# michiyasunaga/qagnn

Measured on NVIDIA B200. Metric: GNN edges/sec, higher is better.
Workload: dtype f32

## Files before the change

### include/qagnn_b200.h

```cpp
#ifndef QAGNN_B200_H_
#define QAGNN_B200_H_

#include <stddef.h>
#include <stdint.h>

#ifdef __cplusplus
extern "C" {
#endif

#define QAGNN_ABI_VERSION 3

enum {
  QAGNN_OK = 0,
  QAGNN_ERR_INVALID_ARGUMENT = -1,
  QAGNN_ERR_CUDA = -2,
  QAGNN_ERR_INDEX_RANGE = -3,
  QAGNN_ERR_WORKSPACE = -4,
  QAGNN_ERR_UNSUPPORTED = -5
};

typedef struct qagnn_shape {
  int64_t N;
  int64_t E;
  int32_t D;
  int32_t H;
  int32_t T;
  int32_t R;
  int32_t k;
  int32_t n_per_graph;
} qagnn_shape;

typedef struct qagnn_edge_encoder_params {
  const float *lin0_w, *lin0_b;
  const float *bn_w, *bn_b, *bn_mean, *bn_var;
  const float *lin3_w, *lin3_b;
} qagnn_edge_encoder_params;

typedef struct qagnn_layer_params {
  const float *key_w, *key_b;
  const float *msg_w, *msg_b;
  const float *query_w, *query_b;
  const float *mlp0_w, *mlp0_b;
  const float *bn_w, *bn_b, *bn_mean, *bn_var;
  const float *mlp3_w, *mlp3_b;
} qagnn_layer_params;

typedef struct qagnn_mp_params {
  const float *emb_node_type_w, *emb_node_type_b;
  const float *emb_score_w, *emb_score_b;
  const float *vh_w, *vh_b, *vx_w, *vx_b;
  const float *score_basis;
} qagnn_mp_params;

int32_t qagnn_abi_version(void);
const char *qagnn_status_string(int32_t status);
const char *qagnn_last_cuda_error(void);


typedef struct qagnn_prep_layout {
  size_t total_bytes;
  size_t src;
  size_t tgt;
  size_t combo;
  size_t rowptr_src;
  size_t rowptr_tgt;
  size_t perm_src;
  size_t perm_tgt;
  size_t csr_src_tgt;
  size_t csr_src_combo;
  size_t csr_tgt_src;
  size_t csr_tgt_combo;
  size_t csr_tgt_apos;
  size_t pk_src;
  size_t pk_tgt;
  size_t csr_src_tpos;
  size_t order_src;
  size_t order_tgt;
  size_t ninfo_src;
  size_t ninfo_tgt;
  size_t status;
  size_t scratch;
} qagnn_prep_layout;

int32_t qagnn_graph_prep_layout(int64_t N, int64_t E, qagnn_prep_layout *out_host);
size_t qagnn_graph_prep_bytes(int64_t N, int64_t E);

int32_t qagnn_graph_prep(const int64_t *edge_index, const int64_t *edge_type, const int64_t *node_type,
                         const qagnn_shape *shape, void *prep, size_t prep_bytes, int32_t validate,
                         void *stream);

int32_t qagnn_graph_prep_packed(const int64_t *edge_index, const int64_t *edge_type, const int64_t *node_type,
                                const int64_t *graph_ptr, int32_t max_edges_per_graph, const qagnn_shape *shape, void *prep,
                                size_t prep_bytes, int32_t validate, void *stream);


size_t qagnn_fold_bytes(const qagnn_shape *shape);
int32_t qagnn_fold_weights(const qagnn_shape *shape, const qagnn_edge_encoder_params *edge_encoder_host,
                           const qagnn_layer_params *layers_host, const qagnn_mp_params *mp_host,
                           void *folded, size_t folded_bytes, void *stream);


size_t qagnn_forward_workspace_bytes(const qagnn_shape *shape);

int32_t qagnn_gatconve_forward(const qagnn_shape *shape, int32_t layer, const float *x, const float *extra,
                               const void *prep, const void *folded, float *out, float *alpha_out,
                               float *aggr_out, void *workspace, size_t workspace_bytes, void *stream);

int32_t qagnn_node_feature_extra(const qagnn_shape *shape, const int64_t *node_type, const float *node_score,
                                 const void *folded, float *extra_out, void *workspace, size_t workspace_bytes,
                                 void *stream);

int32_t qagnn_mp_forward(const qagnn_shape *shape, const float *H_in, const int64_t *node_type,
                         const float *node_score, const void *prep, const void *folded, float *out,
                         float *x_layers_out, void *workspace, size_t workspace_bytes, void *stream);


int32_t qagnn_mp_core_forward(const qagnn_shape *shape, const void *prep, const float *qkm, const float *ke, const float *me,
                              float *aggr, float *alpha_scaled, float *alpha_out, float *scratch, void *stream);

int32_t qagnn_mp_core_backward(const qagnn_shape *shape, const void *prep, const int32_t *combo_order, const float *qkm,
                               const float *ke, const float *me, const float *alpha_scaled, const float *d_aggr,
                               float *d_qkm, float *d_ke, float *d_me, float *scratch, void *stream);

size_t qagnn_linear_workspace_bytes(int64_t M, int32_t N, int32_t K1, int32_t K2);
int32_t qagnn_linear_bf16x3(const float *A1, int32_t lda1, int32_t K1, const float *A2, int32_t lda2, int32_t K2,
                            const float *W, int32_t ldw, const float *bias, float *C, int32_t ldc, int64_t M, int32_t N,
                            int32_t act, void *workspace, size_t workspace_bytes, void *stream);

int32_t qagnn_attention_pool(int32_t B, int32_t n, int32_t D, int32_t n_head, const float *X, const float *qs,
                             const uint8_t *mask, const float *wk, const float *bk, const float *wv, const float *bv,
                             float *pooled, float *attn, void *stream);

int32_t qagnn_decoder_tail(int32_t B, int32_t n, int32_t D, int32_t n_head, int32_t S, const float *X, const float *qs,
                           const int64_t *node_type, const int64_t *adj_lengths, const float *sent_vecs, const float *wk,
                           const float *bk, const float *wv, const float *bv, float *concat, float *attn, void *stream);

int32_t qagnn_decoder_head(int32_t B, int32_t n, int32_t D, const int64_t *concept_ids, int64_t n_concept, const float *table,
                           const float *ctx, const float *node_scores, const int64_t *adj_lengths, float *H_out,
                           float *scores_out, void *stream);

int64_t qagnn_launch_count(void);

enum {
  QAGNN_PROF_GRAPH_PREP = 0,
  QAGNN_PROF_PROJECTION = 1,
  QAGNN_PROF_MESSAGE_PASSING = 2,
  QAGNN_PROF_NODE_MLP = 3,
  QAGNN_PROF_PRO_EPILOGUE = 4,
  QAGNN_PROF_STAGES = 5
};
int32_t qagnn_profile_enable(int32_t on);
int32_t qagnn_profile_read(double *ms_out , int64_t *count_out );

#ifdef __cplusplus
}
#endif
#endif
```

### qagnn_b200/_lib.py

```python
import ctypes as C
import os

import torch

_HERE = os.path.dirname(os.path.abspath(__file__))
LIB_PATH = os.path.join(_HERE, "lib", "libqagnn_b200.so")

OK = 0
STATUS = {0: "ok", -1: "invalid argument", -2: "CUDA error", -3: "index out of range",
          -4: "workspace too small", -5: "unsupported shape"}


class Shape(C.Structure):
    _fields_ = [("N", C.c_int64), ("E", C.c_int64), ("D", C.c_int32), ("H", C.c_int32), ("T", C.c_int32),
                ("R", C.c_int32), ("k", C.c_int32), ("n_per_graph", C.c_int32)]


_P = C.c_void_p


class EdgeEncoderParams(C.Structure):
    _fields_ = [(n, _P) for n in ("lin0_w", "lin0_b", "bn_w", "bn_b", "bn_mean", "bn_var", "lin3_w", "lin3_b")]


class LayerParams(C.Structure):
    _fields_ = [(n, _P) for n in ("key_w", "key_b", "msg_w", "msg_b", "query_w", "query_b", "mlp0_w", "mlp0_b",
                                  "bn_w", "bn_b", "bn_mean", "bn_var", "mlp3_w", "mlp3_b")]


class MPParams(C.Structure):
    _fields_ = [(n, _P) for n in ("emb_node_type_w", "emb_node_type_b", "emb_score_w", "emb_score_b", "vh_w", "vh_b",
                                  "vx_w", "vx_b", "score_basis")]


class PrepLayout(C.Structure):
    _fields_ = [(n, C.c_size_t) for n in ("total_bytes", "src", "tgt", "combo", "rowptr_src", "rowptr_tgt", "perm_src",
                                          "perm_tgt", "csr_src_tgt", "csr_src_combo", "csr_tgt_src", "csr_tgt_combo",
                                          "csr_tgt_apos", "pk_src", "pk_tgt", "csr_src_tpos", "order_src", "order_tgt", "ninfo_src", "ninfo_tgt",
                                          "status", "scratch")]


EXPORTS = {
    "qagnn_abi_version": (C.c_int32, []),
    "qagnn_status_string": (C.c_char_p, [C.c_int32]),
    "qagnn_last_cuda_error": (C.c_char_p, []),
    "qagnn_graph_prep_layout": (C.c_int32, [C.c_int64, C.c_int64, C.POINTER(PrepLayout)]),
    "qagnn_graph_prep_bytes": (C.c_size_t, [C.c_int64, C.c_int64]),
    "qagnn_graph_prep": (C.c_int32, [_P, _P, _P, C.POINTER(Shape), _P, C.c_size_t, C.c_int32, _P]),
    "qagnn_graph_prep_packed": (C.c_int32, [_P, _P, _P, _P, C.c_int32, C.POINTER(Shape), _P, C.c_size_t, C.c_int32, _P]),
    "qagnn_fold_bytes": (C.c_size_t, [C.POINTER(Shape)]),
    "qagnn_fold_weights": (C.c_int32, [C.POINTER(Shape), C.POINTER(EdgeEncoderParams), C.POINTER(LayerParams),
                                       C.POINTER(MPParams), _P, C.c_size_t, _P]),
    "qagnn_forward_workspace_bytes": (C.c_size_t, [C.POINTER(Shape)]),
    "qagnn_gatconve_forward": (C.c_int32, [C.POINTER(Shape), C.c_int32, _P, _P, _P, _P, _P, _P, _P, _P, C.c_size_t, _P]),
    "qagnn_node_feature_extra": (C.c_int32, [C.POINTER(Shape), _P, _P, _P, _P, _P, C.c_size_t, _P]),
    "qagnn_mp_forward": (C.c_int32, [C.POINTER(Shape), _P, _P, _P, _P, _P, _P, _P, _P, C.c_size_t, _P]),
    "qagnn_mp_core_forward": (C.c_int32, [C.POINTER(Shape), _P, _P, _P, _P, _P, _P, _P, _P, _P]),
    "qagnn_mp_core_backward": (C.c_int32, [C.POINTER(Shape), _P, _P, _P, _P, _P, _P, _P, _P, _P, _P, _P, _P]),
    "qagnn_linear_workspace_bytes": (C.c_size_t, [C.c_int64, C.c_int32, C.c_int32, C.c_int32]),
    "qagnn_linear_bf16x3": (C.c_int32, [_P, C.c_int32, C.c_int32, _P, C.c_int32, C.c_int32, _P, C.c_int32, _P, _P, C.c_int32,
                                        C.c_int64, C.c_int32, C.c_int32, _P, C.c_size_t, _P]),
    "qagnn_attention_pool": (C.c_int32, [C.c_int32, C.c_int32, C.c_int32, C.c_int32, _P, _P, _P, _P, _P, _P, _P, _P, _P, _P]),
    "qagnn_decoder_tail": (C.c_int32, [C.c_int32, C.c_int32, C.c_int32, C.c_int32, C.c_int32, _P, _P, _P, _P, _P, _P, _P, _P, _P, _P,
                                       _P, _P]),
    "qagnn_decoder_head": (C.c_int32, [C.c_int32, C.c_int32, C.c_int32, _P, C.c_int64, _P, _P, _P, _P, _P, _P, _P]),
    "qagnn_launch_count": (C.c_int64, []),
    "qagnn_profile_enable": (C.c_int32, [C.c_int32]),
    "qagnn_profile_read": (C.c_int32, [C.POINTER(C.c_double), C.POINTER(C.c_int64)]),
}

_lib = None


def load():
    global _lib
    if _lib is not None:
        return _lib
    from . import build as _build
    if not _build.is_current():
        import fcntl
        stale = os.path.exists(LIB_PATH)
        try:
            _build._nvcc()
        except RuntimeError:
            raise RuntimeError(
                f"{LIB_PATH} is {'older than qagnn_b200/csrc' if stale else 'missing'} and there is no nvcc to build it. Run "
                f"`python -c 'import __graft_entry__ as g; g.build()'` on a machine with the CUDA toolkit. There is no CPU fallback.") from None
        os.makedirs(os.path.dirname(LIB_PATH), exist_ok=True)
        with open(LIB_PATH + ".lock", "w") as lock:
            fcntl.flock(lock, fcntl.LOCK_EX)
            try:
                if not _build.is_current():
                    _build.build()
            except Exception as e:
                raise RuntimeError(f"{LIB_PATH} is {'older than qagnn_b200/csrc' if stale else 'missing'} and could not be "
                                   f"built: {e}. There is no CPU fallback.") from e
            finally:
                fcntl.flock(lock, fcntl.LOCK_UN)
    if not os.path.exists(LIB_PATH):
        raise RuntimeError(f"{LIB_PATH} is missing after a build. There is no CPU fallback.")
    lib = C.CDLL(LIB_PATH)
    for name, (res, args) in EXPORTS.items():
        fn = getattr(lib, name)
        fn.restype, fn.argtypes = res, args
    if lib.qagnn_abi_version() != 3:
        raise RuntimeError("libqagnn_b200.so ABI version mismatch")
    _lib = lib
    return lib


PROF_STAGES = ("graph_prep", "projection", "message_passing", "node_mlp", "pro_epilogue")


def profile_read():
    lib = load()
    ms = (C.c_double * len(PROF_STAGES))()
    cnt = (C.c_int64 * len(PROF_STAGES))()
    check(lib.qagnn_profile_read(ms, cnt), "qagnn_profile_read")
    return {n: (ms[i], cnt[i]) for i, n in enumerate(PROF_STAGES)}


class QagnnError(RuntimeError):
    pass


def check(status, what):
    if status != OK:
        lib = load()
        msg = lib.qagnn_status_string(status).decode()
        if status == -2:
            msg += ": " + lib.qagnn_last_cuda_error().decode()
        if status == -3:
            raise IndexError(f"{what}: {msg}")
        raise QagnnError(f"{what}: {msg} (status {status})")


def ptr(t):
    return None if t is None else C.c_void_p(t.data_ptr())


def stream_ptr(device):
    return C.c_void_p(torch.cuda.current_stream(device).cuda_stream)


def require_cuda(t, name):
    if not t.is_cuda:
        raise RuntimeError(f"qagnn_b200: `{name}` must live on a CUDA device (got {t.device}); "
                           f"this implementation has no CPU path")


def f32c(t, name):
    require_cuda(t, name)
    if t.dtype != torch.float32:
        raise TypeError(f"qagnn_b200: `{name}` must be float32 (got {t.dtype})")
    return t.detach().contiguous()


def i64c(t, name):
    require_cuda(t, name)
    if t.dtype != torch.int64:
        raise TypeError(f"qagnn_b200: `{name}` must be int64 (got {t.dtype})")
    return t.contiguous()
```

### qagnn_b200/csrc/abi.cu

```cuda
#include <atomic>
#include <mutex>
#include <cuda_bf16.h>
#include <stdio.h>
#include <stdlib.h>
#include <string.h>

#include "common.cuh"

namespace qagnn {

static std::atomic<long long> g_launches{0};
static thread_local char g_cuda_err[256] = "";

void note_launch(int n) { g_launches.fetch_add(n, std::memory_order_relaxed); }

int32_t cuda_fail(cudaError_t e, const char* file, int line) {
  const char* base = strrchr(file, '/');
  snprintf(g_cuda_err, sizeof(g_cuda_err), "%s (%s:%d)", cudaGetErrorString(e), base ? base + 1 : file, line);
  return QAGNN_ERR_CUDA;
}

namespace {
constexpr int kProfMax = 8192;
struct ProfState {
  bool on = false;
  int n = 0;
  cudaEvent_t ev[kProfMax][2];
  int created = 0;
  int stage[kProfMax];
  int open_idx[QAGNN_PROF_STAGES];
  std::mutex mu;
} g_prof;
}

void prof_begin(int stage, cudaStream_t st) {
  if (!g_prof.on) return;
  std::lock_guard<std::mutex> lk(g_prof.mu);
  if (!g_prof.on || g_prof.n >= kProfMax) { if (g_prof.on) g_prof.open_idx[stage] = -1; return; }
  const int i = g_prof.n++;
  if (i >= g_prof.created) {
    cudaEventCreate(&g_prof.ev[i][0]);
    cudaEventCreate(&g_prof.ev[i][1]);
    g_prof.created = i + 1;
  }
  g_prof.stage[i] = stage;
  g_prof.open_idx[stage] = i;
  cudaEventRecord(g_prof.ev[i][0], st);
}

void prof_end(int stage, cudaStream_t st) {
  if (!g_prof.on) return;
  std::lock_guard<std::mutex> lk(g_prof.mu);
  const int i = g_prof.open_idx[stage];
  if (i >= 0) cudaEventRecord(g_prof.ev[i][1], st);
}

WorkLayout make_work_layout(const qagnn_shape& s) {
  WorkLayout W;
  const size_t N = (size_t)s.N, D = (size_t)s.D, Ep = (size_t)(s.N + s.E), H = (size_t)s.H;
  size_t o = 0;
  auto take = [&](size_t n) { size_t r = o; o += align_up(n * 4) / 4; return r; };
  const size_t DP = (size_t)head_dim_padded((int)(D / H));
  W.qkm = take(N * 3 * (D > H * DP ? D : H * DP));
  W.aggr = take(N * D);
  W.hmid = take(N * D);
  W.xa = take(N * D);
  W.xb = take(N * D);
  W.extra = take(N * D);
  W.sinb = take(N * (D / 2));
  const size_t half = N * D / 2 + 8;
  W.hp_hi = take(half); W.hp_lo = take(half);
  W.ep_hi = take(half); W.ep_lo = take(half);
  W.xp_hi[0] = take(half); W.xp_lo[0] = take(half);
  W.xp_hi[1] = take(half); W.xp_lo[1] = take(half);
  W.ap_hi = take(half); W.ap_lo = take(half);
  W.mp_hi = take(half); W.mp_lo = take(half);
  const size_t sbh = N * (size_t)round_up8((int)(D / 2)) / 2 + 8;
  W.sb_hi = take(sbh); W.sb_lo = take(sbh);
  const size_t xsh = N * (size_t)round_up8((int)(D + D / 2)) / 2 + 8;
  for (int i = 0; i < 3; ++i) { W.xs_hi[i] = take(xsh); W.xs_lo[i] = take(xsh); }
  const size_t Eps = (Ep + 3) / 4 * 4;
  W.score = take(Eps * H);
  W.alpha = take(Eps * H);
  W.alpha2 = take(2 * Eps * H);
  W.total = o;
  return W;
}

namespace {

__global__ void node_feature_prologue_kernel(int64_t N, int D, int T, const int64_t* __restrict__ node_type,
                                             const float* __restrict__ node_score, const float* __restrict__ type_tab,
                                             const float* __restrict__ basis, float* __restrict__ extra,
                                             float* __restrict__ sinb) {
  const int Dh = D / 2;
  for (int64_t i = blockIdx.x * (int64_t)blockDim.x + threadIdx.x; i < N * Dh; i += (int64_t)gridDim.x * blockDim.x) {
    const int64_t v = i / Dh;
    const int j = (int)(i % Dh);
    int64_t t = node_type[v];
    t = t < 0 ? 0 : (t >= T ? T - 1 : t);
    extra[v * D + j] = type_tab[t * Dh + j];
    sinb[i] = sinf(basis[j] * node_score[v]);
  }
}

__global__ void sin_basis_planes_kernel(int64_t N, int Dh, int ld, const float* __restrict__ node_score,
                                        const float* __restrict__ basis, __nv_bfloat16* __restrict__ hi,
                                        __nv_bfloat16* __restrict__ lo) {
  const int half = Dh / 2;
  for (int64_t i = blockIdx.x * (int64_t)blockDim.x + threadIdx.x; i < N * half; i += (int64_t)gridDim.x * blockDim.x) {
    const int64_t v = i / half;
    const int j = (int)(i % half) * 2;
    const float sc = node_score[v];
    const float a = sinf(basis[j] * sc), b = sinf(basis[j + 1] * sc);
    __nv_bfloat162 h2, l2;
    h2.x = __float2bfloat16_rn(a); h2.y = __float2bfloat16_rn(b);
    l2.x = __float2bfloat16_rn(a - __bfloat162float(h2.x)); l2.y = __float2bfloat16_rn(b - __bfloat162float(h2.y));
    *reinterpret_cast<__nv_bfloat162*>(hi + v * ld + j) = h2;
    *reinterpret_cast<__nv_bfloat162*>(lo + v * ld + j) = l2;
  }
}

__global__ void copy_plane_columns_kernel(int64_t N, int w4, int ld8, const uint2* __restrict__ sh, const uint2* __restrict__ sl,
                                          uint2* __restrict__ d1h, uint2* __restrict__ d1l, uint2* __restrict__ d2h,
                                          uint2* __restrict__ d2l) {
  for (int64_t i = blockIdx.x * (int64_t)blockDim.x + threadIdx.x; i < N * w4; i += (int64_t)gridDim.x * blockDim.x) {
    const int64_t r = i / w4;
    const int c = (int)(i - r * w4);
    const uint2 h = sh[r * ld8 + c], l = sl[r * ld8 + c];
    d1h[r * ld8 + c] = h; d1l[r * ld8 + c] = l;
    d2h[r * ld8 + c] = h; d2l[r * ld8 + c] = l;
  }
}

constexpr int kNfNodes = 64;
__global__ void __launch_bounds__(256) node_feature_fused_kernel(int64_t N, int D, int T, const int64_t* __restrict__ node_type,
                                                                  const float* __restrict__ node_score,
                                                                  const float* __restrict__ type_tab, const float* __restrict__ basis,
                                                                  const float* __restrict__ ws, const float* __restrict__ bs,
                                                                  float* __restrict__ extra, __nv_bfloat16* __restrict__ ex_hi,
                                                                  __nv_bfloat16* __restrict__ ex_lo) {
  extern __shared__ __align__(16) float sm_nf[];
  const int Dh = D / 2;
  float* Wt = sm_nf;
  float* Bt = Wt + (size_t)Dh * Dh;
  const int64_t v0 = (int64_t)blockIdx.x * kNfNodes;
  for (int i = threadIdx.x; i < Dh * Dh; i += 256) Wt[(i % Dh) * Dh + i / Dh] = ws[i];
  for (int i = threadIdx.x; i < kNfNodes * Dh; i += 256) {
    const int k = i / kNfNodes, vi = i % kNfNodes;
    const int64_t v = v0 + vi;
    Bt[i] = v < N ? sinf(basis[k] * node_score[v]) : 0.f;
  }
  __syncthreads();
  auto put4 = [&](int64_t v, int col, const float (&x)[4]) {
    if (extra != nullptr) *reinterpret_cast<float4*>(extra + v * D + col) = make_float4(x[0], x[1], x[2], x[3]);
    if (ex_hi != nullptr) {
      __nv_bfloat16 h[4], l[4];
#pragma unroll
      for (int c = 0; c < 4; ++c) {
        h[c] = __float2bfloat16_rn(x[c]);
        l[c] = __float2bfloat16_rn(x[c] - __bfloat162float(h[c]));
      }
      *reinterpret_cast<uint2*>(ex_hi + v * D + col) = *reinterpret_cast<const uint2*>(h);
      *reinterpret_cast<uint2*>(ex_lo + v * D + col) = *reinterpret_cast<const uint2*>(l);
    }
  };
  const int jg = Dh / 4, ntile = (kNfNodes / 4) * jg;
  for (int tl = threadIdx.x; tl < ntile; tl += 256) {
    const int vi0 = (tl / jg) * 4, j0 = (tl % jg) * 4;
    float acc[4][4];
#pragma unroll
    for (int a = 0; a < 4; ++a)
#pragma unroll
      for (int c = 0; c < 4; ++c) acc[a][c] = 0.f;
    for (int k = 0; k < Dh; ++k) {
      const float4 b = *reinterpret_cast<const float4*>(Bt + k * kNfNodes + vi0);
      const float4 w = *reinterpret_cast<const float4*>(Wt + k * Dh + j0);
      const float bb[4] = {b.x, b.y, b.z, b.w}, ww[4] = {w.x, w.y, w.z, w.w};
#pragma unroll
      for (int a = 0; a < 4; ++a)
#pragma unroll
        for (int c = 0; c < 4; ++c) acc[a][c] = fmaf(bb[a], ww[c], acc[a][c]);
    }
#pragma unroll
    for (int a = 0; a < 4; ++a) {
      const int64_t v = v0 + vi0 + a;
      if (v >= N) continue;
      int64_t t = node_type[v];
      t = t < 0 ? 0 : (t >= T ? T - 1 : t);
      float sc[4], ty[4];
#pragma unroll
      for (int c = 0; c < 4; ++c) {
        sc[c] = gelu_tanh(acc[a][c] + bs[j0 + c]);
        ty[c] = type_tab[t * Dh + j0 + c];
      }
      put4(v, Dh + j0, sc);
      put4(v, j0, ty);
    }
  }
}

int32_t check_shape_fwd(const qagnn_shape* s) {
  if (!s) return QAGNN_ERR_INVALID_ARGUMENT;
  if (s->N <= 0 || s->E < 0 || s->D <= 0 || s->H <= 0 || s->T <= 0 || s->R <= 0 || s->k < 0)
    return QAGNN_ERR_INVALID_ARGUMENT;
  if (s->D % s->H != 0 || s->D % 2 != 0) return QAGNN_ERR_INVALID_ARGUMENT;
  if (s->N + s->E >= (int64_t)1 << 31) return QAGNN_ERR_INVALID_ARGUMENT;
  return QAGNN_OK;
}

bool use_headtile(const qagnn_shape& s) {
  const char* e = getenv("QAGNN_MP_PATH");
  const bool forced = e && (strcmp(e, "csr") == 0 || strcmp(e, "basic") == 0);
  return !forced && headtile_supported(s);
}
bool use_slice(const qagnn_shape& s) {
  const char* e = getenv("QAGNN_MP_PATH");
  return !(e && strcmp(e, "basic") == 0) && slice_supported(s);
}
bool mp_path_supported(const qagnn_shape& s) { return use_headtile(s) || use_slice(s) || basic_mp_supported(s); }

int32_t layer_forward(const qagnn_shape& s, const FoldLayout& L, const WorkLayout& W, int layer, const float* x,
                      const float* extra, const void* prep, const qagnn_prep_layout& pl, const float* folded,
                      float* out, float* alpha_out, float* aggr_out, float* ws, Act final_act, bool tiled,
                      cudaStream_t st) {
  const int D = s.D;
  const float* lb = folded + L.layer0 + (size_t)layer * L.layer_stride;
  float* qkm = ws + W.qkm;
  float* aggr = aggr_out ? aggr_out : ws + W.aggr;
  {
    ProfScope ps(QAGNN_PROF_PROJECTION, st);
    HeadMajorOut hm{tiled ? 1 : 0, D, D / s.H, head_dim_padded(D / s.H), s.H};
    QAGNN_RETURN_IF(sgemm_tn(x, D, D, extra, D, D, lb + L.wp, 2 * D, lb + L.bp, qkm, 3 * D, s.N, 3 * D, ACT_NONE, st, hm));
  }
  {
    ProfScope ps(QAGNN_PROF_MESSAGE_PASSING, st);
    if (tiled) {
      QAGNN_RETURN_IF(launch_message_passing_headtile(s, (const int32_t*)prep, pl, qkm, lb + L.keh, lb + L.meh,
                                                      ws + W.score, ws + W.alpha2, aggr, alpha_out, nullptr, nullptr, st));
    } else if (use_slice(s)) {
      QAGNN_RETURN_IF(launch_message_passing_slice(s, (const int32_t*)prep, pl, qkm, lb + L.ke, lb + L.me, ws + W.score, aggr,
                                                   alpha_out, st));
    } else {
      QAGNN_RETURN_IF(launch_message_passing(s, (const int32_t*)prep, pl, qkm, lb + L.ke, lb + L.me, ws + W.score,
                                             ws + W.alpha, aggr, alpha_out, st));
    }
  }
  {
    ProfScope ps(QAGNN_PROF_NODE_MLP, st);
    QAGNN_RETURN_IF(sgemm_tn(aggr, D, D, nullptr, 0, 0, lb + L.w1, D, lb + L.b1, ws + W.hmid, D, s.N, D, ACT_RELU, st));
    QAGNN_RETURN_IF(sgemm_tn(ws + W.hmid, D, D, nullptr, 0, 0, lb + L.w2, D, lb + L.b2, out, D, s.N, D, final_act, st));
  }
  return QAGNN_OK;
}

bool use_tc(const qagnn_shape& s) { return gemm_tc_available() && s.D % 8 == 0; }

struct Planes {
  const void* hi;
  const void* lo;
  int ld = 0;
};

int32_t layer_forward_tc(const qagnn_shape& s, const FoldLayout& L, const WorkLayout& W, int layer, Planes x, Planes extra,
                         const void* prep, const qagnn_prep_layout& pl, const float* folded, float* out_f32,
                         void* out_hi, void* out_lo, float* alpha_out, float* aggr_out, float* ws, Act final_act,
                         bool tiled, cudaStream_t st, const int64_t* type_bias_classes = nullptr, int out_ldp = 0) {
  const int D = s.D;
  if (out_ldp == 0) out_ldp = D;
  const float* lb = folded + L.layer0 + (size_t)layer * L.layer_stride;
  float* qkm = ws + W.qkm;
  const bool fused_split = tiled && (D / s.H) % 2 == 0;
  float* aggr = aggr_out ? aggr_out : (fused_split ? nullptr : ws + W.aggr);
  {
    ProfScope ps(QAGNN_PROF_PROJECTION, st);
    TcOperand A1{x.hi, x.lo, x.ld ? x.ld : D, D}, A2{extra.hi, extra.lo, D, D};
    TcOutput o{};
    if (tiled && type_bias_classes != nullptr) {
      const int DP = head_dim_padded(D / s.H), KS = round_up8(D + D / 2);
      TcOperand Ax{x.hi, x.lo, KS, D + D / 2}, none{nullptr, nullptr, 0, 0};
      TcOperand Wp{lb + L.wps_hi, lb + L.wps_lo, KS, D + D / 2};
      o.hm_buf = qkm;
      o.hm = HeadMajorOut{1, D, D / s.H, DP, s.H};
      o.row_class = type_bias_classes; o.class_stride = 3 * s.H * DP; o.n_class = s.T;
      QAGNN_RETURN_IF(gemm_tc(Ax, none, Wp, lb + L.tbias, s.N, 3 * s.H * DP, ACT_NONE, o, st));
    } else if (tiled) {
      const int DP = head_dim_padded(D / s.H);
      TcOperand Wp{lb + L.wph_hi, lb + L.wph_lo, 2 * D, 2 * D};
      o.hm_buf = qkm;
      o.hm = HeadMajorOut{1, D, D / s.H, DP, s.H};
      QAGNN_RETURN_IF(gemm_tc(A1, A2, Wp, lb + L.bph, s.N, 3 * s.H * DP, ACT_NONE, o, st));
    } else {
      TcOperand Wp{lb + L.wp_hi, lb + L.wp_lo, 2 * D, 2 * D};
      o.f32 = qkm;
      o.ldc = 3 * D;
      QAGNN_RETURN_IF(gemm_tc(A1, A2, Wp, lb + L.bp, s.N, 3 * D, ACT_NONE, o, st));
    }
  }
  {
    ProfScope ps(QAGNN_PROF_MESSAGE_PASSING, st);
    if (tiled) {
      QAGNN_RETURN_IF(launch_message_passing_headtile(s, (const int32_t*)prep, pl, qkm, lb + L.keh, lb + L.meh,
                                                      ws + W.score, ws + W.alpha2, aggr, alpha_out,
                                                      fused_split ? ws + W.ap_hi : nullptr, ws + W.ap_lo, st));
    } else if (use_slice(s)) {
      QAGNN_RETURN_IF(launch_message_passing_slice(s, (const int32_t*)prep, pl, qkm, lb + L.ke, lb + L.me, ws + W.score, aggr,
                                                   alpha_out, st));
    } else {
      QAGNN_RETURN_IF(launch_message_passing(s, (const int32_t*)prep, pl, qkm, lb + L.ke, lb + L.me, ws + W.score,
                                             ws + W.alpha, aggr, alpha_out, st));
    }
  }
  {
    ProfScope ps(QAGNN_PROF_NODE_MLP, st);
    if (!fused_split) QAGNN_RETURN_IF(split_bf16(aggr, D, s.N, D, ws + W.ap_hi, ws + W.ap_lo, D, st));
    TcOperand A{ws + W.ap_hi, ws + W.ap_lo, D, D}, none{nullptr, nullptr, 0, 0};
    TcOperand W1{lb + L.w1_hi, lb + L.w1_lo, D, D}, W2{lb + L.w2_hi, lb + L.w2_lo, D, D};
    TcOutput o1{};
    o1.hi = ws + W.mp_hi; o1.lo = ws + W.mp_lo; o1.ldp = D;
    QAGNN_RETURN_IF(gemm_tc(A, none, W1, lb + L.b1, s.N, D, ACT_RELU, o1, st));
    TcOperand Hm{ws + W.mp_hi, ws + W.mp_lo, D, D};
    TcOutput o2{};
    o2.f32 = out_f32; o2.ldc = D; o2.hi = out_hi; o2.lo = out_lo; o2.ldp = out_ldp;
    QAGNN_RETURN_IF(gemm_tc(Hm, none, W2, lb + L.b2, s.N, D, final_act, o2, st));
  }
  return QAGNN_OK;
}

int32_t extra_forward(const qagnn_shape& s, const FoldLayout& L, const WorkLayout& W, const int64_t* node_type,
                      const float* node_score, const float* folded, float* extra, float* ws, cudaStream_t st,
                      void* ex_hi = nullptr, void* ex_lo = nullptr) {
  ProfScope ps(QAGNN_PROF_PRO_EPILOGUE, st);
  const int D = s.D, Dh = D / 2;
  if (Dh <= 128 && D % 8 == 0) {
    const size_t smem = ((size_t)Dh * Dh + (size_t)kNfNodes * Dh) * sizeof(float);
    static size_t attr[kMaxDevices] = {0};
    const int dev = current_device();
    if (smem > 48 * 1024 && smem > attr[dev]) {
      QAGNN_CHECK_CUDA(cudaFuncSetAttribute(node_feature_fused_kernel, cudaFuncAttributeMaxDynamicSharedMemorySize, (int)smem));
      attr[dev] = smem;
    }
    node_feature_fused_kernel<<<(unsigned)((s.N + kNfNodes - 1) / kNfNodes), 256, smem, st>>>(
        s.N, D, s.T, node_type, node_score, folded + L.type_tab, folded + L.basis, folded + L.ws, folded + L.bs, extra,
        (__nv_bfloat16*)ex_hi, (__nv_bfloat16*)ex_lo);
    QAGNN_CHECK_LAUNCH();
    return QAGNN_OK;
  }
  const int64_t n = s.N * Dh;
  int64_t g = (n + 255) / 256;
  if (g > 148 * 32) g = 148 * 32;
  node_feature_prologue_kernel<<<(unsigned)g, 256, 0, st>>>(s.N, D, s.T, node_type, node_score, folded + L.type_tab,
                                                            folded + L.basis, extra, ws + W.sinb);
  QAGNN_CHECK_LAUNCH();
  QAGNN_RETURN_IF(sgemm_tn(ws + W.sinb, Dh, Dh, nullptr, 0, 0, folded + L.ws, Dh, folded + L.bs, extra + Dh, D, s.N, Dh,
                           ACT_GELU, st));
  if (ex_hi != nullptr) QAGNN_RETURN_IF(split_bf16(extra, D, s.N, D, ex_hi, ex_lo, D, st));
  return QAGNN_OK;
}

}
}

using namespace qagnn;

extern "C" int32_t qagnn_abi_version(void) { return QAGNN_ABI_VERSION; }

extern "C" const char* qagnn_status_string(int32_t status) {
  switch (status) {
    case QAGNN_OK: return "ok";
    case QAGNN_ERR_INVALID_ARGUMENT: return "invalid argument";
    case QAGNN_ERR_CUDA: return "CUDA error";
    case QAGNN_ERR_INDEX_RANGE: return "index out of range in edge_index / edge_type / node_type";
    case QAGNN_ERR_WORKSPACE: return "workspace too small";
    case QAGNN_ERR_UNSUPPORTED: return "unsupported shape";
    default: return "unknown status";
  }
}

extern "C" const char* qagnn_last_cuda_error(void) { return g_cuda_err; }

extern "C" int64_t qagnn_launch_count(void) { return (int64_t)g_launches.load(std::memory_order_relaxed); }

extern "C" int32_t qagnn_profile_enable(int32_t on) {
  std::lock_guard<std::mutex> lk(g_prof.mu);
  g_prof.on = on != 0;
  g_prof.n = 0;
  for (int i = 0; i < QAGNN_PROF_STAGES; ++i) g_prof.open_idx[i] = -1;
  return QAGNN_OK;
}

extern "C" int32_t qagnn_profile_read(double* ms_out, int64_t* count_out) {
  if (!ms_out || !count_out) return QAGNN_ERR_INVALID_ARGUMENT;
  std::lock_guard<std::mutex> lk(g_prof.mu);
  for (int i = 0; i < QAGNN_PROF_STAGES; ++i) { ms_out[i] = 0.0; count_out[i] = 0; }
  for (int i = 0; i < g_prof.n; ++i) {
    QAGNN_CHECK_CUDA(cudaEventSynchronize(g_prof.ev[i][1]));
    float ms = 0.f;
    QAGNN_CHECK_CUDA(cudaEventElapsedTime(&ms, g_prof.ev[i][0], g_prof.ev[i][1]));
    ms_out[g_prof.stage[i]] += ms;
    count_out[g_prof.stage[i]] += 1;
  }
  return QAGNN_OK;
}

extern "C" size_t qagnn_forward_workspace_bytes(const qagnn_shape* shape) {
  if (check_shape_fwd(shape) != QAGNN_OK) return 0;
  return align_up(make_work_layout(*shape).total * sizeof(float));
}

extern "C" int32_t qagnn_gatconve_forward(const qagnn_shape* shape, int32_t layer, const float* x, const float* extra,
                                          const void* prep, const void* folded, float* out, float* alpha_out,
                                          float* aggr_out, void* workspace, size_t workspace_bytes, void* stream) {
  QAGNN_RETURN_IF(check_shape_fwd(shape));
  if (!x || !extra || !prep || !folded || !out || !workspace) return QAGNN_ERR_INVALID_ARGUMENT;
  if (layer < 0 || layer >= shape->k) return QAGNN_ERR_INVALID_ARGUMENT;
  if (!mp_path_supported(*shape)) return QAGNN_ERR_UNSUPPORTED;
  const FoldLayout L = make_fold_layout(*shape);
  const WorkLayout W = make_work_layout(*shape);
  if (workspace_bytes < W.total * sizeof(float)) return QAGNN_ERR_WORKSPACE;
  qagnn_prep_layout pl;
  QAGNN_RETURN_IF(qagnn_graph_prep_layout(shape->N, shape->E, &pl));
  const bool tiled = use_headtile(*shape);
  cudaStream_t st = (cudaStream_t)stream;
  float* ws = (float*)workspace;
  if (tiled && !use_tc(*shape)) QAGNN_RETURN_IF(zero_head_pads(*shape, ws + W.qkm, st));
  if (use_tc(*shape)) {
    const int D = shape->D;
    QAGNN_RETURN_IF(split_bf16(x, D, shape->N, D, ws + W.xp_hi[0], ws + W.xp_lo[0], D, st));
    QAGNN_RETURN_IF(split_bf16(extra, D, shape->N, D, ws + W.ep_hi, ws + W.ep_lo, D, st));
    return layer_forward_tc(*shape, L, W, layer, Planes{ws + W.xp_hi[0], ws + W.xp_lo[0]}, Planes{ws + W.ep_hi, ws + W.ep_lo},
                            prep, pl, (const float*)folded, out, nullptr, nullptr, alpha_out, aggr_out, ws, ACT_NONE, tiled, st);
  }
  return layer_forward(*shape, L, W, layer, x, extra, prep, pl, (const float*)folded, out, alpha_out, aggr_out, ws,
                       ACT_NONE, tiled, st);
}

extern "C" int32_t qagnn_node_feature_extra(const qagnn_shape* shape, const int64_t* node_type, const float* node_score,
                                            const void* folded, float* extra_out, void* workspace,
                                            size_t workspace_bytes, void* stream) {
  QAGNN_RETURN_IF(check_shape_fwd(shape));
  if (!node_type || !node_score || !folded || !extra_out || !workspace) return QAGNN_ERR_INVALID_ARGUMENT;
  const FoldLayout L = make_fold_layout(*shape);
  const WorkLayout W = make_work_layout(*shape);
  if (workspace_bytes < W.total * sizeof(float)) return QAGNN_ERR_WORKSPACE;
  return extra_forward(*shape, L, W, node_type, node_score, (const float*)folded, extra_out, (float*)workspace,
                       (cudaStream_t)stream);
}

extern "C" int32_t qagnn_mp_forward(const qagnn_shape* shape, const float* H_in, const int64_t* node_type,
                                    const float* node_score, const void* prep, const void* folded, float* out,
                                    float* x_layers_out, void* workspace, size_t workspace_bytes, void* stream) {
  QAGNN_RETURN_IF(check_shape_fwd(shape));
  if (!H_in || !node_type || !node_score || !prep || !folded || !out || !workspace) return QAGNN_ERR_INVALID_ARGUMENT;
  const qagnn_shape& s = *shape;
  if (s.k > 0 && !mp_path_supported(s)) return QAGNN_ERR_UNSUPPORTED;
  const FoldLayout L = make_fold_layout(s);
  const WorkLayout W = make_work_layout(s);
  if (workspace_bytes < W.total * sizeof(float)) return QAGNN_ERR_WORKSPACE;
  qagnn_prep_layout pl;
  QAGNN_RETURN_IF(qagnn_graph_prep_layout(s.N, s.E, &pl));
  cudaStream_t st = (cudaStream_t)stream;
  float* ws = (float*)workspace;
  const float* f = (const float*)folded;
  float* extra = ws + W.extra;
  const bool tc = use_tc(s);
  const bool tiled = use_headtile(s);
  const char* efp = getenv("QAGNN_MP_FASTPROJ");
  const bool fast = tc && tiled && s.k > 0 && (s.D / 2) % 4 == 0 && !(efp && atoi(efp) == 0);
  if (fast) {
    const int D = s.D, Dh = D / 2, KSh = round_up8(Dh), KS = round_up8(D + Dh);
    char* xh[3]; char* xl[3];
    for (int i = 0; i < 3; ++i) { xh[i] = (char*)(ws + W.xs_hi[i]); xl[i] = (char*)(ws + W.xs_lo[i]); }
    {
      ProfScope ps(QAGNN_PROF_PRO_EPILOGUE, st);
      int64_t g = (s.N * (Dh / 2) + 255) / 256;
      if (g > 148 * 32) g = 148 * 32;
      sin_basis_planes_kernel<<<(unsigned)g, 256, 0, st>>>(s.N, Dh, KSh, node_score, f + L.basis, (__nv_bfloat16*)(ws + W.sb_hi),
                                                           (__nv_bfloat16*)(ws + W.sb_lo));
      QAGNN_CHECK_LAUNCH();
      TcOperand A{ws + W.sb_hi, ws + W.sb_lo, KSh, Dh}, none{nullptr, nullptr, 0, 0}, Wsc{f + L.ws_hi, f + L.ws_lo, KSh, Dh};
      TcOutput o{};
      o.hi = xh[0] + (size_t)D * 2; o.lo = xl[0] + (size_t)D * 2; o.ldp = KS;
      QAGNN_RETURN_IF(gemm_tc(A, none, Wsc, f + L.bs, s.N, Dh, ACT_GELU, o, st));
      {
        const int w4 = Dh * 2 / 8, ld8 = KS * 2 / 8;
        int64_t gc = (s.N * w4 + 255) / 256;
        if (gc > 148 * 16) gc = 148 * 16;
        const size_t off = (size_t)D * 2;
        copy_plane_columns_kernel<<<(unsigned)gc, 256, 0, st>>>(s.N, w4, ld8, (const uint2*)(xh[0] + off), (const uint2*)(xl[0] + off),
                                                              (uint2*)(xh[1] + off), (uint2*)(xl[1] + off), (uint2*)(xh[2] + off),
                                                              (uint2*)(xl[2] + off));
        QAGNN_CHECK_LAUNCH();
      }
      QAGNN_RETURN_IF(split_bf16(H_in, D, s.N, D, xh[0], xl[0], KS, st));
    }
    const size_t ND = (size_t)s.N * s.D;
    Planes xin{xh[0], xl[0], KS};
    const Planes ep{nullptr, nullptr, 0};
    for (int l = 0; l < s.k; ++l) {
      float* xo32 = x_layers_out ? x_layers_out + (size_t)l * ND : nullptr;
      void* ohi = xh[1 + (l & 1)];
      void* olo = xl[1 + (l & 1)];
      QAGNN_RETURN_IF(layer_forward_tc(s, L, W, l, xin, ep, prep, pl, f, xo32, ohi, olo, nullptr, nullptr, ws, ACT_GELU, tiled, st,
                                       node_type, KS));
      xin = Planes{ohi, olo, KS};
    }
    ProfScope ps(QAGNN_PROF_PRO_EPILOGUE, st);
    TcOperand A1{xh[0], xl[0], KS, D}, A2{xin.hi, xin.lo, KS, D}, Wv{f + L.vcat_hi, f + L.vcat_lo, 2 * D, 2 * D};
    TcOutput o{};
    o.f32 = out; o.ldc = D;
    return gemm_tc(A1, A2, Wv, f + L.vbias, s.N, D, ACT_GELU, o, st);
  }
  {
    QAGNN_RETURN_IF(extra_forward(s, L, W, node_type, node_score, f, tc && s.D / 2 <= 128 ? nullptr : extra, ws, st,
                                  tc ? ws + W.ep_hi : nullptr, tc ? ws + W.ep_lo : nullptr));
  }
  if (tiled && !use_tc(s)) QAGNN_RETURN_IF(zero_head_pads(s, ws + W.qkm, st));
  const size_t ND = (size_t)s.N * s.D;
  if (tc) {
    const int D = s.D;
    {
      ProfScope ps(QAGNN_PROF_PRO_EPILOGUE, st);
      QAGNN_RETURN_IF(split_bf16(H_in, D, s.N, D, ws + W.hp_hi, ws + W.hp_lo, D, st));
    }
    Planes xin{ws + W.hp_hi, ws + W.hp_lo};
    const Planes ep{ws + W.ep_hi, ws + W.ep_lo};
    for (int l = 0; l < s.k; ++l) {
      float* xo32 = x_layers_out ? x_layers_out + (size_t)l * ND : nullptr;
      void* ohi = ws + W.xp_hi[l & 1];
      void* olo = ws + W.xp_lo[l & 1];
      QAGNN_RETURN_IF(layer_forward_tc(s, L, W, l, xin, ep, prep, pl, f, xo32, ohi, olo, nullptr, nullptr, ws, ACT_GELU,
                                       tiled, st));
      xin = Planes{ohi, olo};
    }
    ProfScope ps(QAGNN_PROF_PRO_EPILOGUE, st);
    TcOperand A1{ws + W.hp_hi, ws + W.hp_lo, D, D}, A2{xin.hi, xin.lo, D, D}, Wv{f + L.vcat_hi, f + L.vcat_lo, 2 * D, 2 * D};
    TcOutput o{};
    o.f32 = out; o.ldc = D;
    if (s.k == 0) { A2 = A1; }
    return gemm_tc(A1, A2, Wv, f + L.vbias, s.N, D, ACT_GELU, o, st);
  }
  const float* x = H_in;
  for (int l = 0; l < s.k; ++l) {
    float* xo = x_layers_out ? x_layers_out + (size_t)l * ND : ws + ((l & 1) ? W.xb : W.xa);
    QAGNN_RETURN_IF(layer_forward(s, L, W, l, x, extra, prep, pl, f, xo, nullptr, nullptr, ws, ACT_GELU, tiled, st));
    x = xo;
  }
  ProfScope ps(QAGNN_PROF_PRO_EPILOGUE, st);
  return sgemm_tn(H_in, s.D, s.D, x, s.D, s.D, f + L.vcat, 2 * s.D, f + L.vbias, out, s.D, s.N, s.D, ACT_GELU, st);
}

extern "C" int32_t qagnn_mp_core_forward(const qagnn_shape* shape, const void* prep, const float* qkm, const float* ke,
                                         const float* me, float* aggr, float* alpha_scaled, float* alpha_out, float* scratch,
                                         void* stream) {
  QAGNN_RETURN_IF(check_shape_fwd(shape));
  if (!prep || !qkm || !ke || !me || !aggr || !alpha_scaled || !scratch) return QAGNN_ERR_INVALID_ARGUMENT;
  qagnn_prep_layout pl;
  QAGNN_RETURN_IF(qagnn_graph_prep_layout(shape->N, shape->E, &pl));
  cudaStream_t st = (cudaStream_t)stream;
  ProfScope ps(QAGNN_PROF_MESSAGE_PASSING, st);
  return launch_message_passing(*shape, (const int32_t*)prep, pl, qkm, ke, me, scratch, alpha_scaled, aggr, alpha_out, st);
}

extern "C" int32_t qagnn_mp_core_backward(const qagnn_shape* shape, const void* prep, const int32_t* combo_order,
                                          const float* qkm, const float* ke, const float* me, const float* alpha_scaled,
                                          const float* d_aggr, float* d_qkm, float* d_ke, float* d_me, float* scratch,
                                          void* stream) {
  QAGNN_RETURN_IF(check_shape_fwd(shape));
  if (!prep || !combo_order || !qkm || !ke || !me || !alpha_scaled || !d_aggr || !d_qkm || !d_ke || !d_me || !scratch)
    return QAGNN_ERR_INVALID_ARGUMENT;
  qagnn_prep_layout pl;
  QAGNN_RETURN_IF(qagnn_graph_prep_layout(shape->N, shape->E, &pl));
  return launch_message_passing_backward(*shape, (const int32_t*)prep, pl, combo_order, qkm, ke, me, alpha_scaled, d_aggr,
                                         scratch, d_qkm, d_ke, d_me, (cudaStream_t)stream);
}

extern "C" size_t qagnn_linear_workspace_bytes(int64_t M, int32_t N, int32_t K1, int32_t K2) {
  if (M <= 0 || N <= 0 || K1 <= 0 || K2 < 0) return 0;
  const size_t K = (size_t)K1 + K2;
  return align_up(2 * 2 * ((size_t)M * K + (size_t)N * K) + 8 * 1024);
}

extern "C" int32_t qagnn_linear_bf16x3(const float* A1, int32_t lda1, int32_t K1, const float* A2, int32_t lda2, int32_t K2,
                                       const float* Wt, int32_t ldw, const float* bias, float* C, int32_t ldc, int64_t M,
                                       int32_t N, int32_t act, void* workspace, size_t workspace_bytes, void* stream) {
  if (!A1 || !Wt || !C || !workspace || M <= 0 || N <= 0 || K1 <= 0 || K2 < 0 || (K2 > 0 && !A2)) return QAGNN_ERR_INVALID_ARGUMENT;
  if (act < 0 || act > 2) return QAGNN_ERR_INVALID_ARGUMENT;
  if (workspace_bytes < qagnn_linear_workspace_bytes(M, N, K1, K2)) return QAGNN_ERR_WORKSPACE;
  if (!gemm_tc_available() || !gemm_tc_shape_ok(K1, K2, K1, K2, K1 + K2, N)) return QAGNN_ERR_UNSUPPORTED;
  cudaStream_t st = (cudaStream_t)stream;
  char* w = (char*)workspace;
  auto take = [&](size_t elems) { char* r = w; w += align_up(elems * 2); return (void*)r; };
  const int K = K1 + K2;
  void *a1h = take((size_t)M * K1), *a1l = take((size_t)M * K1);
  void *a2h = K2 ? take((size_t)M * K2) : nullptr, *a2l = K2 ? take((size_t)M * K2) : nullptr;
  void *wh = take((size_t)N * K), *wl = take((size_t)N * K);
  QAGNN_RETURN_IF(split_bf16(A1, lda1, M, K1, a1h, a1l, K1, st));
  if (K2) QAGNN_RETURN_IF(split_bf16(A2, lda2, M, K2, a2h, a2l, K2, st));
  QAGNN_RETURN_IF(split_bf16(Wt, ldw, N, K, wh, wl, K, st));
  TcOperand o1{a1h, a1l, K1, K1}, o2{a2h, a2l, K2, K2}, ow{wh, wl, K, K};
  TcOutput out{};
  out.f32 = C;
  out.ldc = ldc;
  return gemm_tc(o1, o2, ow, bias, M, N, (Act)act, out, st);
}
```

### qagnn_b200/csrc/common.cuh

```cuda
#pragma once

#include <cuda_runtime.h>
#include <stddef.h>
#include <stdint.h>

#include "../../include/qagnn_b200.h"

namespace qagnn {

constexpr size_t kAlign = 256;
__host__ __device__ inline size_t align_up(size_t x, size_t a = kAlign) { return (x + a - 1) / a * a; }

void note_launch(int n = 1);
int32_t cuda_fail(cudaError_t e, const char* file, int line);

#define QAGNN_CHECK_LAUNCH()                               \
  do {                                                     \
    cudaError_t e__ = cudaGetLastError();                  \
    if (e__ != cudaSuccess) return ::qagnn::cuda_fail(e__, __FILE__, __LINE__);\
    ::qagnn::note_launch();                                \
  } while (0)

#define QAGNN_CHECK_CUDA(expr)                              \
  do {                                                     \
    cudaError_t e__ = (expr);                              \
    if (e__ != cudaSuccess) return ::qagnn::cuda_fail(e__, __FILE__, __LINE__);\
  } while (0)

#define QAGNN_RETURN_IF(st)        \
  do {                             \
    int32_t s__ = (st);            \
    if (s__ != QAGNN_OK) return s__; \
  } while (0)

constexpr int kMaxDevices = 64;
inline int current_device() {
  int dev = 0;
  if (cudaGetDevice(&dev) != cudaSuccess || dev < 0 || dev >= kMaxDevices) dev = 0;
  return dev;
}

void prof_begin(int stage, cudaStream_t st);
void prof_end(int stage, cudaStream_t st);
struct ProfScope {
  int stage; cudaStream_t st;
  ProfScope(int s, cudaStream_t t) : stage(s), st(t) { prof_begin(stage, st); }
  ~ProfScope() { prof_end(stage, st); }
};

struct FoldLayout {
  int D, H, T, R, k, C;
  size_t tab;
  size_t hidden;
  size_t type_tab;
  size_t basis;
  size_t ws;
  size_t bs;
  size_t vcat;
  size_t vbias;
  size_t layer0;
  size_t layer_stride;
  size_t wp;
  size_t bp;
  size_t ke;
  size_t me;
  size_t w1;
  size_t b1;
  size_t w2;
  size_t b2;
  size_t keh;
  size_t meh;
  size_t wp_hi, wp_lo;
  size_t wph, bph;
  size_t wph_hi, wph_lo;
  size_t w1_hi, w1_lo;
  size_t w2_hi, w2_lo;
  size_t vcat_hi, vcat_lo;
  size_t ws_hi, ws_lo;
  size_t wps;
  size_t wps_hi, wps_lo;
  size_t tbias;
  size_t total;
};
FoldLayout make_fold_layout(const qagnn_shape& s);

struct WorkLayout {
  size_t qkm;
  size_t aggr;
  size_t hmid;
  size_t xa, xb;
  size_t extra;
  size_t sinb;
  size_t hp_hi, hp_lo;
  size_t ep_hi, ep_lo;
  size_t xp_hi[2], xp_lo[2];
  size_t ap_hi, ap_lo;
  size_t mp_hi, mp_lo;
  size_t sb_hi, sb_lo;
  size_t xs_hi[3], xs_lo[3];
  size_t score;
  size_t alpha;
  size_t alpha2;
  size_t total;
};
WorkLayout make_work_layout(const qagnn_shape& s);

enum Act { ACT_NONE = 0, ACT_RELU = 1, ACT_GELU = 2 };

struct HeadMajorOut {
  int enabled, D, d, DP, H;
};

int32_t sgemm_tn(const float* A1, int lda1, int K1, const float* A2, int lda2, int K2, const float* W, int ldw,
                 const float* bias, float* C, int ldc, int64_t M, int N, Act act, cudaStream_t st,
                 HeadMajorOut hm = HeadMajorOut{0, 0, 0, 0, 0});

struct TcOperand {
  const void* hi;
  const void* lo;
  int ld, K;
};
struct TcOutput {
  float* f32; int ldc;
  float* hm_buf; HeadMajorOut hm;
  void* hi; void* lo; int ldp;
  const int64_t* row_class; int class_stride; int n_class;
};
bool gemm_tc_available();
bool gemm_tc_shape_ok(int K1, int K2, int lda1, int lda2, int ldw, int N);
int32_t split_bf16(const float* a, int lda, long long M, int K, void* hi, void* lo, int ldp, cudaStream_t st);
int32_t gemm_tc(const TcOperand& A1, const TcOperand& A2, const TcOperand& W, const float* bias, long long M, int N,
                Act act, const TcOutput& out, cudaStream_t st);

inline int head_dim_padded(int d) { return (d + 3) / 4 * 4; }
inline int round_up8(int k) { return (k + 7) / 8 * 8; }
bool headtile_supported(const qagnn_shape& s);
int32_t launch_message_passing_headtile(const qagnn_shape& s, const int32_t* prep_base, const qagnn_prep_layout& pl,
                                        const float* qkmh, const float* keh, const float* meh, float* score,
                                        float* alpha2, float* aggr, float* alpha_out, void* aggr_hi, void* aggr_lo,
                                        cudaStream_t st);
int32_t zero_head_pads(const qagnn_shape& s, float* qkmh, cudaStream_t st);

bool basic_mp_supported(const qagnn_shape& s);
int32_t launch_message_passing(const qagnn_shape& s, const int32_t* prep_base, const qagnn_prep_layout& pl,
                               const float* qkm, const float* ke, const float* me, float* score, float* alpha,
                               float* aggr, float* alpha_out, cudaStream_t st);

bool slice_supported(const qagnn_shape& s);
int32_t launch_message_passing_slice(const qagnn_shape& s, const int32_t* prep_base, const qagnn_prep_layout& pl,
                                     const float* qkm, const float* ke, const float* me, float* score, float* aggr,
                                     float* alpha_out, cudaStream_t st);

int32_t launch_message_passing_backward(const qagnn_shape& s, const int32_t* prep_base, const qagnn_prep_layout& pl,
                                        const int32_t* combo_order, const float* qkm, const float* ke, const float* me,
                                        const float* alpha_s, const float* d_aggr, float* ds, float* d_qkm, float* d_ke,
                                        float* d_me, cudaStream_t st);

__device__ __forceinline__ float gelu_tanh(float x) {
  const float k0 = 0.7978845608028654f;
  return 0.5f * x * (1.0f + tanhf(k0 * (x + 0.044715f * x * x * x)));
}

}
```

### qagnn_b200/csrc/gemm_tc.cu

```cuda
#include <cuda.h>
#include <cuda_bf16.h>
#include <stdio.h>
#include <stdlib.h>
#include <string.h>

#include "common.cuh"

namespace qagnn {

namespace {

constexpr int BM = 128;
constexpr int kEpiWarps = 8;
constexpr int kThreads = (kEpiWarps + 2) * 32;
constexpr int kTmaWarp = kEpiWarps, kMmaWarp = kEpiWarps + 1;

struct alignas(64) TcParams {
  CUtensorMap a_hi[2], a_lo[2], w_hi, w_lo;
  CUtensorMap o_f32, o_hm, o_hi, o_lo;
  int nseg, kseg[2];
  int umma_n, n_step, N, stages;
  int nkb_total;
  long long M;
  const float* bias;
  const int64_t* row_class;
  int class_stride, n_class;
  int act;
  float* c_f32;
  int ldc;
  float* c_hm;
  HeadMajorOut hm;
  __nv_bfloat16 *c_hi, *c_lo;
  int ldp;
  unsigned tmem_cols;
};

__device__ __forceinline__ uint32_t smem_u32(const void* p) { return (uint32_t)__cvta_generic_to_shared(p); }

__device__ __forceinline__ void mbar_init(uint64_t* bar, uint32_t count) {
  asm volatile("mbarrier.init.shared::cta.b64 [%0], %1;" ::"r"(smem_u32(bar)), "r"(count) : "memory");
}
__device__ __forceinline__ void mbar_expect_tx(uint64_t* bar, uint32_t bytes) {
  asm volatile("mbarrier.arrive.expect_tx.shared::cta.b64 _, [%0], %1;" ::"r"(smem_u32(bar)), "r"(bytes) : "memory");
}
__device__ __forceinline__ void mbar_wait(uint64_t* bar, uint32_t parity) {
  uint32_t done;
  do {
    asm volatile(
        "{\n\t.reg .pred p;\n\t"
        "mbarrier.try_wait.parity.shared::cta.b64 p, [%1], %2;\n\t"
        "selp.u32 %0, 1, 0, p;\n\t}"
        : "=r"(done)
        : "r"(smem_u32(bar)), "r"(parity)
        : "memory");
  } while (!done);
}
__device__ __forceinline__ void tma_load_2d(void* dst, const CUtensorMap* map, int c0, int c1, uint64_t* bar) {
  asm volatile(
      "cp.async.bulk.tensor.2d.shared::cluster.global.tile.mbarrier::complete_tx::bytes [%0], [%1, {%2, %3}], [%4];" ::"r"(
          smem_u32(dst)),
      "l"(map), "r"(c0), "r"(c1), "r"(smem_u32(bar))
      : "memory");
}
__device__ __forceinline__ void tc_fence_before() { asm volatile("tcgen05.fence::before_thread_sync;" ::: "memory"); }
__device__ __forceinline__ void tc_fence_after() { asm volatile("tcgen05.fence::after_thread_sync;" ::: "memory"); }

template <int BK>
__device__ __forceinline__ uint64_t umma_desc(uint32_t saddr) {
  const uint32_t lo = ((saddr & 0x3FFFFu) >> 4) | (1u << 16);
  const uint32_t hi = (uint32_t)(8 * BK * 2 / 16) | (1u << 14) | ((BK == 64 ? 2u : 4u) << 29);
  return ((uint64_t)hi << 32) | lo;
}
__device__ __forceinline__ void umma_bf16(uint32_t tmem_d, uint64_t da, uint64_t db, uint32_t idesc, uint32_t acc) {
  asm volatile(
      "{\n\t.reg .pred p;\n\t"
      "setp.ne.b32 p, %4, 0;\n\t"
      "tcgen05.mma.cta_group::1.kind::f16 [%0], %1, %2, %3, p;\n\t}" ::"r"(tmem_d),
      "l"(da), "l"(db), "r"(idesc), "r"(acc)
      : "memory");
}
__device__ __forceinline__ void umma_commit(uint64_t* bar) {
  asm volatile("tcgen05.commit.cta_group::1.mbarrier::arrive::one.shared::cluster.b64 [%0];" ::"r"(smem_u32(bar)) : "memory");
}
__device__ __forceinline__ void tmem_ld32(uint32_t taddr, float (&v)[32]) {
  uint32_t r[32];
  asm volatile(
      "tcgen05.ld.sync.aligned.32x32b.x32.b32 "
      "{%0,%1,%2,%3,%4,%5,%6,%7,%8,%9,%10,%11,%12,%13,%14,%15,%16,%17,%18,%19,%20,%21,%22,%23,%24,%25,%26,%27,%28,%29,%30,%31}, [%32];"
      : "=r"(r[0]), "=r"(r[1]), "=r"(r[2]), "=r"(r[3]), "=r"(r[4]), "=r"(r[5]), "=r"(r[6]), "=r"(r[7]), "=r"(r[8]),
        "=r"(r[9]), "=r"(r[10]), "=r"(r[11]), "=r"(r[12]), "=r"(r[13]), "=r"(r[14]), "=r"(r[15]), "=r"(r[16]), "=r"(r[17]),
        "=r"(r[18]), "=r"(r[19]), "=r"(r[20]), "=r"(r[21]), "=r"(r[22]), "=r"(r[23]), "=r"(r[24]), "=r"(r[25]), "=r"(r[26]),
        "=r"(r[27]), "=r"(r[28]), "=r"(r[29]), "=r"(r[30]), "=r"(r[31])
      : "r"(taddr));
  asm volatile("tcgen05.wait::ld.sync.aligned;" ::: "memory");
#pragma unroll
  for (int i = 0; i < 32; ++i) v[i] = __uint_as_float(r[i]);
}

__device__ __forceinline__ float gelu_tanh_fast(float x) {
  const float u = 0.7978845608028654f * (x + 0.044715f * x * x * x);
  const float t = 1.f - __fdividef(2.f, __expf(2.f * u) + 1.f);
  return 0.5f * x * (1.f + t);
}

constexpr int kStageBytesPerWarp = 4096;

__device__ __forceinline__ void tma_store_2d(const CUtensorMap* map, int c0, int c1, const void* src) {
  asm volatile("cp.async.bulk.tensor.2d.global.shared::cta.tile.bulk_group [%0, {%1, %2}], [%3];" ::"l"(map), "r"(c0), "r"(c1),
               "r"(smem_u32(src))
               : "memory");
}
__device__ __forceinline__ void tma_store_3d(const CUtensorMap* map, int c0, int c1, int c2, const void* src) {
  asm volatile("cp.async.bulk.tensor.3d.global.shared::cta.tile.bulk_group [%0, {%1, %2, %3}], [%4];" ::"l"(map), "r"(c0),
               "r"(c1), "r"(c2), "r"(smem_u32(src))
               : "memory");
}
__device__ __forceinline__ void tma_store_commit() { asm volatile("cp.async.bulk.commit_group;" ::: "memory"); }
__device__ __forceinline__ void tma_store_wait_read() { asm volatile("cp.async.bulk.wait_group.read 0;" ::: "memory"); }
__device__ __forceinline__ void tma_store_wait_all() { asm volatile("cp.async.bulk.wait_group 0;" ::: "memory"); }

constexpr uint32_t kPeerBitMask = 0xFEFFFFFFu;
__device__ __forceinline__ uint32_t cluster_ctarank() {
  uint32_t r;
  asm volatile("mov.u32 %0, %%cluster_ctarank;" : "=r"(r));
  return r;
}
__device__ __forceinline__ void cluster_sync_all() {
  asm volatile("barrier.cluster.arrive.release.aligned;" ::: "memory");
  asm volatile("barrier.cluster.wait.acquire.aligned;" ::: "memory");
}
__device__ __forceinline__ void tma_load_2d_2sm(void* dst, const CUtensorMap* map, int c0, int c1, uint64_t* bar) {
  asm volatile(
      "cp.async.bulk.tensor.2d.cta_group::2.shared::cluster.global.mbarrier::complete_tx::bytes [%0], [%1, {%2, %3}], [%4];" ::"r"(
          smem_u32(dst)),
      "l"(map), "r"(c0), "r"(c1), "r"(smem_u32(bar) & kPeerBitMask)
      : "memory");
}
__device__ __forceinline__ void umma_bf16_2sm(uint32_t tmem_d, uint64_t da, uint64_t db, uint32_t idesc, uint32_t acc) {
  asm volatile(
      "{\n\t.reg .pred p;\n\t"
      "setp.ne.b32 p, %4, 0;\n\t"
      "tcgen05.mma.cta_group::2.kind::f16 [%0], %1, %2, %3, p;\n\t}" ::"r"(tmem_d),
      "l"(da), "l"(db), "r"(idesc), "r"(acc)
      : "memory");
}
__device__ __forceinline__ void umma_commit_2sm(uint64_t* bar) {
  asm volatile("tcgen05.commit.cta_group::2.mbarrier::arrive::one.shared::cluster.multicast::cluster.b64 [%0], %1;" ::"r"(smem_u32(bar)),
               "h"((uint16_t)3)
               : "memory");
}
__device__ __forceinline__ void mbar_arrive_leader(uint64_t* bar) {
  asm volatile("mbarrier.arrive.shared::cluster.b64 _, [%0];" ::"r"(smem_u32(bar) & kPeerBitMask) : "memory");
}

template <int ACT, int BK, int CTAS, bool WRES>
__global__ void __launch_bounds__(kThreads, 1) gemm_tc_kernel(const __grid_constant__ TcParams p) {
  extern __shared__ __align__(1024) unsigned char smem[];
  const int warp = threadIdx.x >> 5, lane = threadIdx.x & 31;
  const uint32_t a_bytes = BM * BK * 2;
  const uint32_t wn = (uint32_t)p.umma_n / CTAS;
  const uint32_t w_bytes = wn * BK * 2;
  const uint32_t stage_bytes = WRES ? 2 * a_bytes : 2 * a_bytes + 2 * w_bytes;
  const uint32_t rank = CTAS == 2 ? cluster_ctarank() : 0u;
  const bool leader = rank == 0;
  const unsigned cl_id = blockIdx.x / CTAS, n_cl = gridDim.x / CTAS;
  const uint32_t wres_bytes = WRES ? (uint32_t)p.nkb_total * 2u * w_bytes : 0u;
  unsigned char* wres = smem + (size_t)p.stages * stage_bytes;
  unsigned char* ctrl = wres + wres_bytes;
  uint64_t* full = reinterpret_cast<uint64_t*>(ctrl);
  uint64_t* empty = full + p.stages;
  uint64_t* acc_full = empty + p.stages;
  uint64_t* acc_empty = acc_full + 2;
  uint64_t* wfull = acc_empty + 2;
  uint32_t* tmem_slot = reinterpret_cast<uint32_t*>(wfull + 1);

  int nkb_seg[2];
  nkb_seg[0] = (p.kseg[0] + BK - 1) / BK;
  nkb_seg[1] = p.nseg > 1 ? (p.kseg[1] + BK - 1) / BK : 0;
  const int nkb = nkb_seg[0] + nkb_seg[1];
  const int n_tiles = (p.N + p.n_step - 1) / p.n_step;
  const long long m_tiles = (p.M + BM * CTAS - 1) / (BM * CTAS);
  const long long total_tiles = m_tiles * n_tiles;
  const int my_n = WRES ? (int)(cl_id % (unsigned)n_tiles) : 0;
  const long long w_idx = cl_id / (unsigned)n_tiles;
  const long long w_cnt = WRES ? ((long long)n_cl - my_n + n_tiles - 1) / n_tiles : 1;
  const long long t_first = WRES ? w_idx * n_tiles + my_n : (long long)cl_id;
  const long long t_step = WRES ? w_cnt * n_tiles : (long long)n_cl;

  if (threadIdx.x == 0) {
    for (int s = 0; s < p.stages; ++s) {
      mbar_init(&full[s], 1);
      mbar_init(&empty[s], 1);
    }
    for (int a = 0; a < 2; ++a) {
      mbar_init(&acc_full[a], 1);
      mbar_init(&acc_empty[a], kEpiWarps * CTAS);
    }
    mbar_init(wfull, 1);
    asm volatile("fence.mbarrier_init.release.cluster;" ::: "memory");
  }
  if (warp == kMmaWarp) {
    if (CTAS == 1) {
      asm volatile("tcgen05.alloc.cta_group::1.sync.aligned.shared::cta.b32 [%0], %1;" ::"r"(smem_u32(tmem_slot)), "r"(512u) : "memory");
      asm volatile("tcgen05.relinquish_alloc_permit.cta_group::1.sync.aligned;" ::: "memory");
    } else {
      asm volatile("tcgen05.alloc.cta_group::2.sync.aligned.shared::cta.b32 [%0], %1;" ::"r"(smem_u32(tmem_slot)), "r"(512u) : "memory");
      asm volatile("tcgen05.relinquish_alloc_permit.cta_group::2.sync.aligned;" ::: "memory");
    }
  }
  tc_fence_before();
  __syncthreads();
  if (CTAS == 2) cluster_sync_all();
  tc_fence_after();
  const uint32_t tmem_base = *tmem_slot;

  if (warp == kTmaWarp) {
    if (lane == 0) {
      long long it = 0;
      if (WRES && t_first < total_tiles) {
        const int n0 = my_n * p.n_step + (int)(rank * wn);
        if (CTAS == 1) mbar_expect_tx(wfull, wres_bytes);
        else if (leader) mbar_expect_tx(wfull, 2 * wres_bytes);
        for (int kb = 0; kb < nkb; ++kb) {
          unsigned char* dst = wres + (size_t)kb * 2 * w_bytes;
          if (CTAS == 1) {
            tma_load_2d(dst, &p.w_hi, kb * BK, n0, wfull);
            tma_load_2d(dst + w_bytes, &p.w_lo, kb * BK, n0, wfull);
          } else {
            tma_load_2d_2sm(dst, &p.w_hi, kb * BK, n0, wfull);
            tma_load_2d_2sm(dst + w_bytes, &p.w_lo, kb * BK, n0, wfull);
          }
        }
      }
      for (long long tile = t_first; tile < total_tiles; tile += t_step) {
        const int n0 = (int)(tile % n_tiles) * p.n_step + (int)(rank * wn);
        const int m0 = (int)((tile / n_tiles) * BM * CTAS + rank * BM);
        for (int kb = 0; kb < nkb; ++kb, ++it) {
          const int s = (int)(it % p.stages);
          if (it >= p.stages) mbar_wait(&empty[s], (uint32_t)((it / p.stages) - 1) & 1u);
          const int seg = kb < nkb_seg[0] ? 0 : 1;
          const int k_in_seg = (seg == 0 ? kb : kb - nkb_seg[0]) * BK;
          const int k_glob = (seg == 0 ? 0 : p.kseg[0]) + k_in_seg;
          unsigned char* st = smem + (size_t)s * stage_bytes;
          if (WRES) {
            if (CTAS == 1) {
              mbar_expect_tx(&full[s], stage_bytes);
              tma_load_2d(st, &p.a_hi[0], k_in_seg, m0, &full[s]);
              tma_load_2d(st + a_bytes, &p.a_lo[0], k_in_seg, m0, &full[s]);
            } else {
              if (leader) mbar_expect_tx(&full[s], 2 * stage_bytes);
              tma_load_2d_2sm(st, &p.a_hi[0], k_in_seg, m0, &full[s]);
              tma_load_2d_2sm(st + a_bytes, &p.a_lo[0], k_in_seg, m0, &full[s]);
            }
          } else if (CTAS == 1) {
            mbar_expect_tx(&full[s], stage_bytes);
            tma_load_2d(st, &p.a_hi[seg], k_in_seg, m0, &full[s]);
            tma_load_2d(st + a_bytes, &p.a_lo[seg], k_in_seg, m0, &full[s]);
            tma_load_2d(st + 2 * a_bytes, &p.w_hi, k_glob, n0, &full[s]);
            tma_load_2d(st + 2 * a_bytes + w_bytes, &p.w_lo, k_glob, n0, &full[s]);
          } else {
            if (leader) mbar_expect_tx(&full[s], 2 * stage_bytes);
            tma_load_2d_2sm(st, &p.a_hi[seg], k_in_seg, m0, &full[s]);
            tma_load_2d_2sm(st + a_bytes, &p.a_lo[seg], k_in_seg, m0, &full[s]);
            tma_load_2d_2sm(st + 2 * a_bytes, &p.w_hi, k_glob, n0, &full[s]);
            tma_load_2d_2sm(st + 2 * a_bytes + w_bytes, &p.w_lo, k_glob, n0, &full[s]);
          }
        }
      }
    }
  } else if (warp == kMmaWarp) {
    if (lane == 0 && leader) {
      const uint32_t idesc = (1u << 4) | (1u << 7) | (1u << 10) | ((uint32_t)(p.umma_n >> 3) << 17) | ((uint32_t)((BM * CTAS) >> 4) << 24);
      long long it = 0;
      int ti = 0;
      if (WRES && t_first < total_tiles) {
        mbar_wait(wfull, 0);
        tc_fence_after();
      }
      for (long long tile = t_first; tile < total_tiles; tile += t_step, ++ti) {
        const int acc = ti & 1;
        if (ti >= 2) {
          mbar_wait(&acc_empty[acc], (uint32_t)((ti >> 1) - 1) & 1u);
          tc_fence_after();
        }
        const uint32_t tmem_d = tmem_base + (uint32_t)acc * 256u;
        for (int kb = 0; kb < nkb; ++kb, ++it) {
          const int s = (int)(it % p.stages);
          mbar_wait(&full[s], (uint32_t)(it / p.stages) & 1u);
          tc_fence_after();
          const int seg = kb < nkb_seg[0] ? 0 : 1;
          const int k_in_seg = (seg == 0 ? kb : kb - nkb_seg[0]) * BK;
          const int krem = p.kseg[seg] - k_in_seg;
          const int nsteps = krem >= BK ? BK / 16 : (krem + 15) / 16;
          const uint32_t sa = smem_u32(smem + (size_t)s * stage_bytes);
          for (int k = 0; k < nsteps; ++k) {
            const uint64_t da_hi = umma_desc<BK>(sa + k * 32), da_lo = umma_desc<BK>(sa + a_bytes + k * 32);
            const uint32_t sw = WRES ? smem_u32(wres + (size_t)kb * 2 * w_bytes) : sa + 2 * a_bytes;
            const uint64_t dw_hi = umma_desc<BK>(sw + k * 32), dw_lo = umma_desc<BK>(sw + w_bytes + k * 32);
            if (CTAS == 1) {
              umma_bf16(tmem_d, da_hi, dw_hi, idesc, (kb | k) != 0);
              umma_bf16(tmem_d, da_hi, dw_lo, idesc, 1u);
              umma_bf16(tmem_d, da_lo, dw_hi, idesc, 1u);
            } else {
              umma_bf16_2sm(tmem_d, da_hi, dw_hi, idesc, (kb | k) != 0);
              umma_bf16_2sm(tmem_d, da_hi, dw_lo, idesc, 1u);
              umma_bf16_2sm(tmem_d, da_lo, dw_hi, idesc, 1u);
            }
          }
          if (CTAS == 1) umma_commit(&empty[s]);
          else umma_commit_2sm(&empty[s]);
        }
        if (CTAS == 1) umma_commit(&acc_full[acc]);
        else umma_commit_2sm(&acc_full[acc]);
      }
    }
  } else {
    const int quad = warp & 3;
    unsigned char* stg = ctrl + 1024 + (size_t)warp * kStageBytesPerWarp;
    const bool hm_mode = p.c_hm != nullptr;
    const int DP = hm_mode ? p.hm.DP : 0;
    const int per_head = hm_mode ? (DP + 31) / 32 : 0;
    const int nblk = hm_mode ? p.hm.H * per_head : (p.n_step + 31) / 32;
    int ti = 0;
    for (long long tile = t_first; tile < total_tiles; tile += t_step, ++ti) {
      const int acc = ti & 1;
      const int n_tile = (int)(tile % n_tiles);
      const int n0 = n_tile * p.n_step;
      const int row0 = (int)((tile / n_tiles) * BM * CTAS + rank * BM) + quad * 32;
      const float* bias_row = p.bias;
      if (p.row_class != nullptr) {
        const long long r = (long long)row0 + lane;
        long long c = r < p.M ? p.row_class[r] : 0;
        c = c < 0 ? 0 : (c >= p.n_class ? p.n_class - 1 : c);
        bias_row = p.bias + (size_t)c * p.class_stride;
      }
      mbar_wait(&acc_full[acc], (uint32_t)(ti >> 1) & 1u);
      tc_fence_after();
      const uint32_t taddr = tmem_base + (uint32_t)acc * 256u + ((uint32_t)(quad * 32) << 16);
      for (int blk = warp >> 2; blk < nblk; blk += kEpiWarps / 4) {
        int tcol, oc0, oslab = 0;
        if (hm_mode) {
          const int hh = blk / per_head, q = blk % per_head;
          tcol = hh * DP + 32 * q;
          oc0 = 32 * q;
          oslab = n_tile * p.hm.H + hh;
        } else {
          tcol = 32 * blk;
          oc0 = n0 + tcol;
          if (oc0 >= p.N) break;
        }
        float v[32];
        tmem_ld32(taddr + (uint32_t)tcol, v);
        if (p.bias != nullptr) {
          if (n0 + tcol + 32 <= p.N) {
            const float4* b4 = reinterpret_cast<const float4*>(bias_row + n0 + tcol);
#pragma unroll
            for (int i = 0; i < 8; ++i) {
              const float4 b = __ldg(b4 + i);
              v[4 * i] += b.x; v[4 * i + 1] += b.y; v[4 * i + 2] += b.z; v[4 * i + 3] += b.w;
            }
          } else {
#pragma unroll
            for (int i = 0; i < 32; ++i)
              if (n0 + tcol + i < p.N) v[i] += __ldg(bias_row + n0 + tcol + i);
          }
        }
#pragma unroll
        for (int i = 0; i < 32; ++i) {
          if (ACT == ACT_RELU) v[i] = fmaxf(v[i], 0.f);
          if (ACT == ACT_GELU) v[i] = gelu_tanh_fast(v[i]);
        }
        if (p.c_f32 != nullptr || hm_mode) {
          tma_store_wait_read();
          __syncwarp();
#pragma unroll
          for (int c = 0; c < 8; ++c)
            *reinterpret_cast<float4*>(stg + lane * 128 + ((c ^ (lane & 7)) << 4)) = make_float4(v[4 * c], v[4 * c + 1], v[4 * c + 2], v[4 * c + 3]);
          asm volatile("fence.proxy.async.shared::cta;" ::: "memory");
          __syncwarp();
          if (lane == 0) {
            if (hm_mode) tma_store_3d(&p.o_hm, oc0, row0, oslab, stg);
            else tma_store_2d(&p.o_f32, oc0, row0, stg);
            tma_store_commit();
          }
        }
        if (p.c_hi != nullptr) {
          tma_store_wait_read();
          __syncwarp();
          uint32_t hi[16], lo[16];
#pragma unroll
          for (int i = 0; i < 16; ++i) {
            __nv_bfloat162 h2, l2;
            h2.x = __float2bfloat16_rn(v[2 * i]);
            h2.y = __float2bfloat16_rn(v[2 * i + 1]);
            l2.x = __float2bfloat16_rn(v[2 * i] - __bfloat162float(h2.x));
            l2.y = __float2bfloat16_rn(v[2 * i + 1] - __bfloat162float(h2.y));
            hi[i] = *reinterpret_cast<uint32_t*>(&h2);
            lo[i] = *reinterpret_cast<uint32_t*>(&l2);
          }
#pragma unroll
          for (int c = 0; c < 4; ++c) {
            const int off = lane * 64 + ((c ^ ((lane >> 1) & 3)) << 4);
            *reinterpret_cast<uint4*>(stg + off) = make_uint4(hi[4 * c], hi[4 * c + 1], hi[4 * c + 2], hi[4 * c + 3]);
            *reinterpret_cast<uint4*>(stg + 2048 + off) = make_uint4(lo[4 * c], lo[4 * c + 1], lo[4 * c + 2], lo[4 * c + 3]);
          }
          asm volatile("fence.proxy.async.shared::cta;" ::: "memory");
          __syncwarp();
          if (lane == 0) {
            tma_store_2d(&p.o_hi, oc0, row0, stg);
            tma_store_2d(&p.o_lo, oc0, row0, stg + 2048);
            tma_store_commit();
          }
        }
      }
      tc_fence_before();
      __syncwarp();
      if (lane == 0) {
        if (CTAS == 1) asm volatile("mbarrier.arrive.shared::cta.b64 _, [%0];" ::"r"(smem_u32(&acc_empty[acc])) : "memory");
        else mbar_arrive_leader(&acc_empty[acc]);
      }
    }
    tma_store_wait_all();
  }
  tc_fence_before();
  __syncthreads();
  if (CTAS == 2) cluster_sync_all();
  if (warp == kMmaWarp) {
    tc_fence_after();
    if (CTAS == 1) asm volatile("tcgen05.dealloc.cta_group::1.sync.aligned.b32 %0, %1;" ::"r"(tmem_base), "r"(512u) : "memory");
    else asm volatile("tcgen05.dealloc.cta_group::2.sync.aligned.b32 %0, %1;" ::"r"(tmem_base), "r"(512u) : "memory");
  }
}

__global__ void split_bf16_kernel(const float* __restrict__ a, int lda, long long M, int K, __nv_bfloat16* __restrict__ hi,
                                  __nv_bfloat16* __restrict__ lo, int ldp) {
  const long long total = M * (long long)(K / 2);
  for (long long i = blockIdx.x * (long long)blockDim.x + threadIdx.x; i < total; i += (long long)gridDim.x * blockDim.x) {
    const long long r = i / (K / 2);
    const int c = (int)(i % (K / 2)) * 2;
    const float2 v = *reinterpret_cast<const float2*>(a + r * lda + c);
    const __nv_bfloat16 h0 = __float2bfloat16_rn(v.x), h1 = __float2bfloat16_rn(v.y);
    __nv_bfloat162 hh, ll;
    hh.x = h0; hh.y = h1;
    ll.x = __float2bfloat16_rn(v.x - __bfloat162float(h0));
    ll.y = __float2bfloat16_rn(v.y - __bfloat162float(h1));
    *reinterpret_cast<__nv_bfloat162*>(hi + r * ldp + c) = hh;
    *reinterpret_cast<__nv_bfloat162*>(lo + r * ldp + c) = ll;
  }
}

typedef CUresult (*EncodeTiledFn)(CUtensorMap*, CUtensorMapDataType, cuuint32_t, void*, const cuuint64_t*, const cuuint64_t*,
                                  const cuuint32_t*, const cuuint32_t*, CUtensorMapInterleave, CUtensorMapSwizzle,
                                  CUtensorMapL2promotion, CUtensorMapFloatOOBfill);

EncodeTiledFn encode_fn() {
  static EncodeTiledFn fn = [] {
    void* f = nullptr;
    cudaDriverEntryPointQueryResult q;
    if (cudaGetDriverEntryPoint("cuTensorMapEncodeTiled", &f, cudaEnableDefault, &q) != cudaSuccess ||
        q != cudaDriverEntryPointSuccess)
      f = nullptr;
    return (EncodeTiledFn)f;
  }();
  return fn;
}

bool make_map(CUtensorMap* m, const void* base, long long rows, int K, int ld, int box_rows, int BK) {
  EncodeTiledFn enc = encode_fn();
  if (!enc) return false;
  cuuint64_t dims[2] = {(cuuint64_t)K, (cuuint64_t)rows};
  cuuint64_t strides[1] = {(cuuint64_t)ld * 2};
  cuuint32_t box[2] = {(cuuint32_t)BK, (cuuint32_t)box_rows};
  cuuint32_t estr[2] = {1, 1};
  return enc(m, CU_TENSOR_MAP_DATA_TYPE_BFLOAT16, 2, const_cast<void*>(base), dims, strides, box, estr,
             CU_TENSOR_MAP_INTERLEAVE_NONE, BK == 64 ? CU_TENSOR_MAP_SWIZZLE_128B : CU_TENSOR_MAP_SWIZZLE_64B,
             CU_TENSOR_MAP_L2_PROMOTION_L2_128B,
             CU_TENSOR_MAP_FLOAT_OOB_FILL_NONE) == CUDA_SUCCESS;
}

bool make_out_map(CUtensorMap* m, void* base, int elem_bytes, long long cols, long long rows, long long slabs,
                  size_t row_stride_bytes, size_t slab_stride_bytes) {
  EncodeTiledFn enc = encode_fn();
  if (!enc) return false;
  cuuint64_t dims[3] = {(cuuint64_t)cols, (cuuint64_t)rows, (cuuint64_t)(slabs > 0 ? slabs : 1)};
  cuuint64_t strides[2] = {(cuuint64_t)row_stride_bytes, (cuuint64_t)slab_stride_bytes};
  cuuint32_t box[3] = {32, 32, 1};
  cuuint32_t estr[3] = {1, 1, 1};
  const int rank = slabs > 0 ? 3 : 2;
  return enc(m, elem_bytes == 4 ? CU_TENSOR_MAP_DATA_TYPE_FLOAT32 : CU_TENSOR_MAP_DATA_TYPE_BFLOAT16, rank, base, dims, strides,
             box, estr, CU_TENSOR_MAP_INTERLEAVE_NONE, elem_bytes == 4 ? CU_TENSOR_MAP_SWIZZLE_128B : CU_TENSOR_MAP_SWIZZLE_64B,
             CU_TENSOR_MAP_L2_PROMOTION_NONE, CU_TENSOR_MAP_FLOAT_OOB_FILL_NONE) == CUDA_SUCCESS;
}

}

bool gemm_tc_available() {
  const char* e = getenv("QAGNN_GEMM");
  const bool forced_off = e && strcmp(e, "ffma") == 0;
  return !forced_off && encode_fn() != nullptr;
}

bool gemm_tc_shape_ok(int K1, int K2, int lda1, int lda2, int ldw, int N) {
  return K1 > 0 && K1 % 2 == 0 && K2 >= 0 && lda1 % 8 == 0 && (K2 == 0 || lda2 % 8 == 0) && ldw % 8 == 0 && N >= 8;
}

int32_t split_bf16(const float* a, int lda, long long M, int K, void* hi, void* lo, int ldp, cudaStream_t st) {
  if (M <= 0 || K <= 0) return QAGNN_OK;
  if (K % 2 != 0 || lda % 2 != 0) return QAGNN_ERR_UNSUPPORTED;
  long long g = (M * (K / 2) + 255) / 256;
  if (g > 148 * 32) g = 148 * 32;
  split_bf16_kernel<<<(unsigned)g, 256, 0, st>>>(a, lda, M, K, (__nv_bfloat16*)hi, (__nv_bfloat16*)lo, ldp);
  QAGNN_CHECK_LAUNCH();
  return QAGNN_OK;
}

int32_t gemm_tc(const TcOperand& A1, const TcOperand& A2, const TcOperand& W, const float* bias, long long M, int N, Act act,
                const TcOutput& out, cudaStream_t st) {
  if (M <= 0 || N <= 0) return QAGNN_OK;
  if (!gemm_tc_available()) return QAGNN_ERR_UNSUPPORTED;
  const int K1 = A1.K, K2 = A2.hi ? A2.K : 0;
  if (!gemm_tc_shape_ok(K1, K2, A1.ld, A2.ld, W.ld, N)) return QAGNN_ERR_UNSUPPORTED;
  TcParams p;
  memset(&p, 0, sizeof(p));
  int n_tiles = (N + 223) / 224;
  p.n_step = (N + n_tiles - 1) / n_tiles;
  p.n_step = (p.n_step + 31) / 32 * 32;
  if (out.hm_buf != nullptr) {
    p.n_step = out.hm.H * out.hm.DP;
    if (p.n_step > 256 || p.n_step % 16 != 0 || N % p.n_step != 0) return QAGNN_ERR_UNSUPPORTED;
    n_tiles = N / p.n_step;
  }
  p.umma_n = (p.n_step + 15) / 16 * 16;
  p.N = N;
  p.M = M;
  p.nseg = K2 > 0 ? 2 : 1;
  p.kseg[0] = K1;
  p.kseg[1] = K2;
  p.tmem_cols = 512;
  const char* e2 = getenv("QAGNN_TC_2CTA");
  const int CTAS = (e2 && atoi(e2) == 0) ? 1 : 2;
  constexpr int BK = 64;
  const size_t smem_cap = 227 * 1024, epi_bytes = kEpiWarps * (size_t)kStageBytesPerWarp;
  const size_t w_blk = (size_t)(p.umma_n / CTAS) * BK * 2;
  const int nkb1 = (K1 + BK - 1) / BK;
  const char* ewr = getenv("QAGNN_TC_WRES");
  bool wres = K2 == 0 && CTAS == 2 && (ewr && atoi(ewr) == 1);
  size_t stage_bytes = 2 * (size_t)BM * BK * 2 + 2 * w_blk;
  size_t wres_bytes = 0;
  int stages = 0;
  if (wres) {
    wres_bytes = (size_t)nkb1 * 2 * w_blk;
    const size_t a_stage = 2 * (size_t)BM * BK * 2;
    if (wres_bytes + 2 * a_stage + 1024 + epi_bytes > smem_cap) { wres = false; wres_bytes = 0; }
    else {
      stage_bytes = a_stage;
      stages = (int)((smem_cap - 1024 - epi_bytes - wres_bytes) / a_stage);
    }
  }
  if (!wres) stages = (int)((226 * 1024 - 1024 - epi_bytes) / stage_bytes);
  if (stages > 6) stages = 6;
  if (stages < 2) return QAGNN_ERR_UNSUPPORTED;
  p.stages = stages;
  p.nkb_total = nkb1;
  const size_t smem_bytes = stages * stage_bytes + wres_bytes + 1024 + epi_bytes;
  bool ok = make_map(&p.a_hi[0], A1.hi, M, K1, A1.ld, BM, BK) && make_map(&p.a_lo[0], A1.lo, M, K1, A1.ld, BM, BK);
  if (K2 > 0) ok = ok && make_map(&p.a_hi[1], A2.hi, M, K2, A2.ld, BM, BK) && make_map(&p.a_lo[1], A2.lo, M, K2, A2.ld, BM, BK);
  ok = ok && make_map(&p.w_hi, W.hi, N, K1 + K2, W.ld, p.umma_n / CTAS, BK) &&
       make_map(&p.w_lo, W.lo, N, K1 + K2, W.ld, p.umma_n / CTAS, BK);
  if (out.f32 != nullptr) ok = ok && make_out_map(&p.o_f32, out.f32, 4, N, M, 0, (size_t)out.ldc * 4, 0);
  if (out.hm_buf != nullptr)
    ok = ok && make_out_map(&p.o_hm, out.hm_buf, 4, out.hm.DP, M, N / p.n_step * out.hm.H, (size_t)out.hm.DP * 4,
                            (size_t)M * out.hm.DP * 4);
  if (out.hi != nullptr)
    ok = ok && make_out_map(&p.o_hi, out.hi, 2, N, M, 0, (size_t)out.ldp * 2, 0) &&
         make_out_map(&p.o_lo, out.lo, 2, N, M, 0, (size_t)out.ldp * 2, 0);
  if (!ok) return QAGNN_ERR_CUDA;
  if ((out.f32 && (out.ldc % 4 != 0)) || (out.hi && (out.ldp % 8 != 0))) return QAGNN_ERR_UNSUPPORTED;
  p.bias = bias;
  p.row_class = bias != nullptr ? out.row_class : nullptr;
  p.class_stride = out.class_stride;
  p.n_class = out.n_class > 0 ? out.n_class : 1;
  p.act = (int)act;
  p.c_f32 = out.f32;
  p.ldc = out.ldc;
  p.c_hm = out.hm_buf;
  p.hm = out.hm;
  p.c_hi = (__nv_bfloat16*)out.hi;
  p.c_lo = (__nv_bfloat16*)out.lo;
  p.ldp = out.ldp;
  static size_t attr_c[kMaxDevices] = {0};
  const int dev_i = current_device();
  size_t& attr = attr_c[dev_i];
  if (attr == 0) {
#define QAGNN_SET_ATTR(A, B, Cn) \
  QAGNN_CHECK_CUDA(cudaFuncSetAttribute(gemm_tc_kernel<A, B, Cn, false>, cudaFuncAttributeMaxDynamicSharedMemorySize, (int)(226 * 1024)))
    QAGNN_SET_ATTR(ACT_NONE, 64, 1); QAGNN_SET_ATTR(ACT_RELU, 64, 1); QAGNN_SET_ATTR(ACT_GELU, 64, 1);
    QAGNN_SET_ATTR(ACT_NONE, 64, 2); QAGNN_SET_ATTR(ACT_RELU, 64, 2); QAGNN_SET_ATTR(ACT_GELU, 64, 2);
#undef QAGNN_SET_ATTR
#define QAGNN_SET_ATTR_W(A) \
  QAGNN_CHECK_CUDA(cudaFuncSetAttribute(gemm_tc_kernel<A, 64, 2, true>, cudaFuncAttributeMaxDynamicSharedMemorySize, (int)smem_cap))
    QAGNN_SET_ATTR_W(ACT_NONE); QAGNN_SET_ATTR_W(ACT_RELU); QAGNN_SET_ATTR_W(ACT_GELU);
#undef QAGNN_SET_ATTR_W
    attr = smem_bytes;
  }
  static int sms_c[kMaxDevices] = {0};
  if (sms_c[dev_i] == 0) QAGNN_CHECK_CUDA(cudaDeviceGetAttribute(&sms_c[dev_i], cudaDevAttrMultiProcessorCount, dev_i));
  const int sms = sms_c[dev_i];
  const long long total_tiles = (long long)n_tiles * ((M + (long long)BM * CTAS - 1) / ((long long)BM * CTAS));
  long long units = total_tiles < sms / CTAS ? total_tiles : sms / CTAS;
  if (wres && units < n_tiles) units = n_tiles;
  const unsigned grid = (unsigned)(units * CTAS);
  cudaLaunchConfig_t cfg;
  memset(&cfg, 0, sizeof(cfg));
  cfg.gridDim = dim3(grid);
  cfg.blockDim = dim3(kThreads);
  cfg.dynamicSmemBytes = smem_bytes;
  cfg.stream = st;
  cudaLaunchAttribute lattr[1];
  lattr[0].id = cudaLaunchAttributeClusterDimension;
  lattr[0].val.clusterDim.x = CTAS;
  lattr[0].val.clusterDim.y = 1;
  lattr[0].val.clusterDim.z = 1;
  cfg.attrs = lattr;
  cfg.numAttrs = CTAS == 2 ? 1 : 0;
  if (getenv("QAGNN_DEBUG")) fprintf(stderr, "gemm_tc: M=%lld N=%d K1=%d K2=%d act=%d wres=%d CTAS=%d stages=%d smem=%zu grid=%u umma_n=%d n_tiles=%d\n", M, N, K1, K2, (int)act, (int)wres, CTAS, stages, smem_bytes, grid, p.umma_n, n_tiles);
#define QAGNN_LAUNCH(A)                                                                          \
  do {                                                                                           \
    if (wres) QAGNN_CHECK_CUDA(cudaLaunchKernelEx(&cfg, gemm_tc_kernel<A, 64, 2, true>, p));               \
    else if (CTAS == 2) QAGNN_CHECK_CUDA(cudaLaunchKernelEx(&cfg, gemm_tc_kernel<A, 64, 2, false>, p));    \
    else QAGNN_CHECK_CUDA(cudaLaunchKernelEx(&cfg, gemm_tc_kernel<A, 64, 1, false>, p));                   \
  } while (0)
  if (act == ACT_NONE) QAGNN_LAUNCH(ACT_NONE);
  else if (act == ACT_RELU) QAGNN_LAUNCH(ACT_RELU);
  else QAGNN_LAUNCH(ACT_GELU);
#undef QAGNN_LAUNCH
  QAGNN_CHECK_LAUNCH();
  return QAGNN_OK;
}

}
```

### qagnn_b200/ops.py

```python
import torch

from . import _lib


def linear_bf16x3(a1, weight, bias=None, a2=None, act="none"):
    lib = _lib.load()
    a1 = _lib.f32c(a1, "a1")
    w = _lib.f32c(weight, "weight")
    a2c = _lib.f32c(a2, "a2") if a2 is not None else None
    b = _lib.f32c(bias, "bias") if bias is not None else None
    M, K1 = a1.shape
    K2 = a2c.shape[1] if a2c is not None else 0
    N = w.shape[0]
    if w.shape[1] != K1 + K2:
        raise ValueError("weight must be [N, K1+K2]")
    out = torch.empty(M, N, dtype=torch.float32, device=a1.device)
    nbytes = lib.qagnn_linear_workspace_bytes(M, N, K1, K2)
    ws = torch.empty(nbytes, dtype=torch.uint8, device=a1.device)
    code = {"none": 0, "relu": 1, "gelu": 2}[act]
    with torch.cuda.device(a1.device):
        st = lib.qagnn_linear_bf16x3(_lib.ptr(a1), K1, K1, _lib.ptr(a2c), K2, K2, _lib.ptr(w), K1 + K2, _lib.ptr(b),
                                     _lib.ptr(out), N, M, N, code, _lib.ptr(ws), nbytes, _lib.stream_ptr(a1.device))
    _lib.check(st, "qagnn_linear_bf16x3")
    return out
```

Baseline: 1.046 billion.

## Fuse node MLP's two tensor-core GEMMs into one kernel keeping hidden on-chip

Adds a dedicated node-MLP kernel that computes Linear-ReLU-Linear in a single tcgen05 launch, keeping the hidden activation on chip (TMEM/shared) instead of writing bf16 hi/lo planes to global memory and reloading them. The forward path uses it when D fits the fused limit, and falls back to a two-launch path with workspace otherwise. Shared device helpers move into a common header. This removes one launch and one full M×D round trip through HBM per layer, at the cost of a more complex kernel with a D limit and higher shared-memory/TMEM pressure.

```diff
diff --git a/include/qagnn_b200.h b/include/qagnn_b200.h
--- a/include/qagnn_b200.h
+++ b/include/qagnn_b200.h
@@ -127,6 +127,11 @@
                             const float *W, int32_t ldw, const float *bias, float *C, int32_t ldc, int64_t M, int32_t N,
                             int32_t act, void *workspace, size_t workspace_bytes, void *stream);
 
+size_t qagnn_node_mlp_workspace_bytes(int64_t M, int32_t D);
+int32_t qagnn_node_mlp_bf16x3(const float *A, int32_t lda, const float *W1, const float *b1, const float *W2, const float *b2,
+                              float *C, int32_t ldc, int64_t M, int32_t D, int32_t act, void *workspace, size_t workspace_bytes,
+                              void *stream);
+
 int32_t qagnn_attention_pool(int32_t B, int32_t n, int32_t D, int32_t n_head, const float *X, const float *qs,
                              const uint8_t *mask, const float *wk, const float *bk, const float *wv, const float *bv,
                              float *pooled, float *attn, void *stream);
diff --git a/qagnn_b200/_lib.py b/qagnn_b200/_lib.py
--- a/qagnn_b200/_lib.py
+++ b/qagnn_b200/_lib.py
@@ -60,6 +60,9 @@
     "qagnn_linear_workspace_bytes": (C.c_size_t, [C.c_int64, C.c_int32, C.c_int32, C.c_int32]),
     "qagnn_linear_bf16x3": (C.c_int32, [_P, C.c_int32, C.c_int32, _P, C.c_int32, C.c_int32, _P, C.c_int32, _P, _P, C.c_int32,
                                         C.c_int64, C.c_int32, C.c_int32, _P, C.c_size_t, _P]),
+    "qagnn_node_mlp_workspace_bytes": (C.c_size_t, [C.c_int64, C.c_int32]),
+    "qagnn_node_mlp_bf16x3": (C.c_int32, [_P, C.c_int32, _P, _P, _P, _P, _P, C.c_int32, C.c_int64, C.c_int32, C.c_int32, _P,
+                                          C.c_size_t, _P]),
     "qagnn_attention_pool": (C.c_int32, [C.c_int32, C.c_int32, C.c_int32, C.c_int32, _P, _P, _P, _P, _P, _P, _P, _P, _P, _P]),
     "qagnn_decoder_tail": (C.c_int32, [C.c_int32, C.c_int32, C.c_int32, C.c_int32, C.c_int32, _P, _P, _P, _P, _P, _P, _P, _P, _P, _P,
                                        _P, _P]),
diff --git a/qagnn_b200/csrc/abi.cu b/qagnn_b200/csrc/abi.cu
--- a/qagnn_b200/csrc/abi.cu
+++ b/qagnn_b200/csrc/abi.cu
@@ -74,7 +74,8 @@
   W.xp_hi[0] = take(half); W.xp_lo[0] = take(half);
   W.xp_hi[1] = take(half); W.xp_lo[1] = take(half);
   W.ap_hi = take(half); W.ap_lo = take(half);
-  W.mp_hi = take(half); W.mp_lo = take(half);
+  const size_t mlp_half = node_mlp_fused_fits((int)D) ? 0 : half;
+  W.mp_hi = take(mlp_half); W.mp_lo = take(mlp_half);
   const size_t sbh = N * (size_t)round_up8((int)(D / 2)) / 2 + 8;
   W.sb_hi = take(sbh); W.sb_lo = take(sbh);
   const size_t xsh = N * (size_t)round_up8((int)(D + D / 2)) / 2 + 8;
@@ -314,15 +315,13 @@
   {
     ProfScope ps(QAGNN_PROF_NODE_MLP, st);
     if (!fused_split) QAGNN_RETURN_IF(split_bf16(aggr, D, s.N, D, ws + W.ap_hi, ws + W.ap_lo, D, st));
-    TcOperand A{ws + W.ap_hi, ws + W.ap_lo, D, D}, none{nullptr, nullptr, 0, 0};
+    TcOperand A{ws + W.ap_hi, ws + W.ap_lo, D, D};
     TcOperand W1{lb + L.w1_hi, lb + L.w1_lo, D, D}, W2{lb + L.w2_hi, lb + L.w2_lo, D, D};
-    TcOutput o1{};
-    o1.hi = ws + W.mp_hi; o1.lo = ws + W.mp_lo; o1.ldp = D;
-    QAGNN_RETURN_IF(gemm_tc(A, none, W1, lb + L.b1, s.N, D, ACT_RELU, o1, st));
-    TcOperand Hm{ws + W.mp_hi, ws + W.mp_lo, D, D};
-    TcOutput o2{};
-    o2.f32 = out_f32; o2.ldc = D; o2.hi = out_hi; o2.lo = out_lo; o2.ldp = out_ldp;
-    QAGNN_RETURN_IF(gemm_tc(Hm, none, W2, lb + L.b2, s.N, D, final_act, o2, st));
+    TcOutput o{};
+    o.f32 = out_f32; o.ldc = D; o.hi = out_hi; o.lo = out_lo; o.ldp = out_ldp;
+    const bool two_launch = !node_mlp_fused_fits(D);
+    QAGNN_RETURN_IF(node_mlp_tc(A, W1, lb + L.b1, W2, lb + L.b2, s.N, D, final_act, o, two_launch ? ws + W.mp_hi : nullptr,
+                                two_launch ? ws + W.mp_lo : nullptr, st));
   }
   return QAGNN_OK;
 }
@@ -604,3 +603,34 @@
   out.ldc = ldc;
   return gemm_tc(o1, o2, ow, bias, M, N, (Act)act, out, st);
 }
+
+extern "C" size_t qagnn_node_mlp_workspace_bytes(int64_t M, int32_t D) {
+  if (M <= 0 || D <= 0) return 0;
+  const size_t a = align_up((size_t)M * D * 2), w = align_up((size_t)D * D * 2);
+  return align_up(2 * a + 4 * w + (node_mlp_fused_fits(D) ? 0 : 2 * a) + 8 * 1024);
+}
+
+extern "C" int32_t qagnn_node_mlp_bf16x3(const float* A, int32_t lda, const float* W1, const float* b1, const float* W2,
+                                         const float* b2, float* C, int32_t ldc, int64_t M, int32_t D, int32_t act,
+                                         void* workspace, size_t workspace_bytes, void* stream) {
+  if (!A || !W1 || !b1 || !W2 || !b2 || !C || !workspace || M <= 0 || D <= 0 || lda < D || ldc < D) return QAGNN_ERR_INVALID_ARGUMENT;
+  if (act < 0 || act > 2) return QAGNN_ERR_INVALID_ARGUMENT;
+  if (workspace_bytes < qagnn_node_mlp_workspace_bytes(M, D)) return QAGNN_ERR_WORKSPACE;
+  if (!gemm_tc_available() || D % 8 != 0 || ldc % 4 != 0) return QAGNN_ERR_UNSUPPORTED;
+  cudaStream_t st = (cudaStream_t)stream;
+  char* w = (char*)workspace;
+  auto take = [&](size_t elems) { char* r = w; w += align_up(elems * 2); return (void*)r; };
+  void *ah = take((size_t)M * D), *al = take((size_t)M * D);
+  void *w1h = take((size_t)D * D), *w1l = take((size_t)D * D), *w2h = take((size_t)D * D), *w2l = take((size_t)D * D);
+  const bool two_launch = !node_mlp_fused_fits(D);
+  void* hh = two_launch ? take((size_t)M * D) : nullptr;
+  void* hl = two_launch ? take((size_t)M * D) : nullptr;
+  QAGNN_RETURN_IF(split_bf16(A, lda, M, D, ah, al, D, st));
+  QAGNN_RETURN_IF(split_bf16(W1, D, D, D, w1h, w1l, D, st));
+  QAGNN_RETURN_IF(split_bf16(W2, D, D, D, w2h, w2l, D, st));
+  TcOperand a{ah, al, D, D}, o1{w1h, w1l, D, D}, o2{w2h, w2l, D, D};
+  TcOutput out{};
+  out.f32 = C;
+  out.ldc = ldc;
+  return node_mlp_tc(a, o1, b1, o2, b2, M, D, (Act)act, out, hh, hl, st);
+}
diff --git a/qagnn_b200/csrc/common.cuh b/qagnn_b200/csrc/common.cuh
--- a/qagnn_b200/csrc/common.cuh
+++ b/qagnn_b200/csrc/common.cuh
@@ -132,6 +132,10 @@
 int32_t gemm_tc(const TcOperand& A1, const TcOperand& A2, const TcOperand& W, const float* bias, long long M, int N,
                 Act act, const TcOutput& out, cudaStream_t st);
 
+bool node_mlp_fused_fits(int D);
+int32_t node_mlp_tc(const TcOperand& A, const TcOperand& W1, const float* b1, const TcOperand& W2, const float* b2, long long M,
+                    int D, Act act2, const TcOutput& out, void* hid_hi, void* hid_lo, cudaStream_t st);
+
 inline int head_dim_padded(int d) { return (d + 3) / 4 * 4; }
 inline int round_up8(int k) { return (k + 7) / 8 * 8; }
 bool headtile_supported(const qagnn_shape& s);
diff --git a/qagnn_b200/csrc/gemm_tc.cu b/qagnn_b200/csrc/gemm_tc.cu
--- a/qagnn_b200/csrc/gemm_tc.cu
+++ b/qagnn_b200/csrc/gemm_tc.cu
@@ -1,10 +1,8 @@
-#include <cuda.h>
-#include <cuda_bf16.h>
 #include <stdio.h>
 #include <stdlib.h>
 #include <string.h>
 
-#include "common.cuh"
+#include "tc_sm100.cuh"
 
 namespace qagnn {
 
@@ -34,124 +32,6 @@
   int ldp;
   unsigned tmem_cols;
 };
-
-__device__ __forceinline__ uint32_t smem_u32(const void* p) { return (uint32_t)__cvta_generic_to_shared(p); }
-
-__device__ __forceinline__ void mbar_init(uint64_t* bar, uint32_t count) {
-  asm volatile("mbarrier.init.shared::cta.b64 [%0], %1;" ::"r"(smem_u32(bar)), "r"(count) : "memory");
-}
-__device__ __forceinline__ void mbar_expect_tx(uint64_t* bar, uint32_t bytes) {
-  asm volatile("mbarrier.arrive.expect_tx.shared::cta.b64 _, [%0], %1;" ::"r"(smem_u32(bar)), "r"(bytes) : "memory");
-}
-__device__ __forceinline__ void mbar_wait(uint64_t* bar, uint32_t parity) {
-  uint32_t done;
-  do {
-    asm volatile(
-        "{\n\t.reg .pred p;\n\t"
-        "mbarrier.try_wait.parity.shared::cta.b64 p, [%1], %2;\n\t"
-        "selp.u32 %0, 1, 0, p;\n\t}"
-        : "=r"(done)
-        : "r"(smem_u32(bar)), "r"(parity)
-        : "memory");
-  } while (!done);
-}
-__device__ __forceinline__ void tma_load_2d(void* dst, const CUtensorMap* map, int c0, int c1, uint64_t* bar) {
-  asm volatile(
-      "cp.async.bulk.tensor.2d.shared::cluster.global.tile.mbarrier::complete_tx::bytes [%0], [%1, {%2, %3}], [%4];" ::"r"(
-          smem_u32(dst)),
-      "l"(map), "r"(c0), "r"(c1), "r"(smem_u32(bar))
-      : "memory");
-}
-__device__ __forceinline__ void tc_fence_before() { asm volatile("tcgen05.fence::before_thread_sync;" ::: "memory"); }
-__device__ __forceinline__ void tc_fence_after() { asm volatile("tcgen05.fence::after_thread_sync;" ::: "memory"); }
-
-template <int BK>
-__device__ __forceinline__ uint64_t umma_desc(uint32_t saddr) {
-  const uint32_t lo = ((saddr & 0x3FFFFu) >> 4) | (1u << 16);
-  const uint32_t hi = (uint32_t)(8 * BK * 2 / 16) | (1u << 14) | ((BK == 64 ? 2u : 4u) << 29);
-  return ((uint64_t)hi << 32) | lo;
-}
-__device__ __forceinline__ void umma_bf16(uint32_t tmem_d, uint64_t da, uint64_t db, uint32_t idesc, uint32_t acc) {
-  asm volatile(
-      "{\n\t.reg .pred p;\n\t"
-      "setp.ne.b32 p, %4, 0;\n\t"
-      "tcgen05.mma.cta_group::1.kind::f16 [%0], %1, %2, %3, p;\n\t}" ::"r"(tmem_d),
-      "l"(da), "l"(db), "r"(idesc), "r"(acc)
-      : "memory");
-}
-__device__ __forceinline__ void umma_commit(uint64_t* bar) {
-  asm volatile("tcgen05.commit.cta_group::1.mbarrier::arrive::one.shared::cluster.b64 [%0];" ::"r"(smem_u32(bar)) : "memory");
-}
-__device__ __forceinline__ void tmem_ld32(uint32_t taddr, float (&v)[32]) {
-  uint32_t r[32];
-  asm volatile(
-      "tcgen05.ld.sync.aligned.32x32b.x32.b32 "
-      "{%0,%1,%2,%3,%4,%5,%6,%7,%8,%9,%10,%11,%12,%13,%14,%15,%16,%17,%18,%19,%20,%21,%22,%23,%24,%25,%26,%27,%28,%29,%30,%31}, [%32];"
-      : "=r"(r[0]), "=r"(r[1]), "=r"(r[2]), "=r"(r[3]), "=r"(r[4]), "=r"(r[5]), "=r"(r[6]), "=r"(r[7]), "=r"(r[8]),
-        "=r"(r[9]), "=r"(r[10]), "=r"(r[11]), "=r"(r[12]), "=r"(r[13]), "=r"(r[14]), "=r"(r[15]), "=r"(r[16]), "=r"(r[17]),
-        "=r"(r[18]), "=r"(r[19]), "=r"(r[20]), "=r"(r[21]), "=r"(r[22]), "=r"(r[23]), "=r"(r[24]), "=r"(r[25]), "=r"(r[26]),
-        "=r"(r[27]), "=r"(r[28]), "=r"(r[29]), "=r"(r[30]), "=r"(r[31])
-      : "r"(taddr));
-  asm volatile("tcgen05.wait::ld.sync.aligned;" ::: "memory");
-#pragma unroll
-  for (int i = 0; i < 32; ++i) v[i] = __uint_as_float(r[i]);
-}
-
-__device__ __forceinline__ float gelu_tanh_fast(float x) {
-  const float u = 0.7978845608028654f * (x + 0.044715f * x * x * x);
-  const float t = 1.f - __fdividef(2.f, __expf(2.f * u) + 1.f);
-  return 0.5f * x * (1.f + t);
-}
-
-constexpr int kStageBytesPerWarp = 4096;
-
-__device__ __forceinline__ void tma_store_2d(const CUtensorMap* map, int c0, int c1, const void* src) {
-  asm volatile("cp.async.bulk.tensor.2d.global.shared::cta.tile.bulk_group [%0, {%1, %2}], [%3];" ::"l"(map), "r"(c0), "r"(c1),
-               "r"(smem_u32(src))
-               : "memory");
-}
-__device__ __forceinline__ void tma_store_3d(const CUtensorMap* map, int c0, int c1, int c2, const void* src) {
-  asm volatile("cp.async.bulk.tensor.3d.global.shared::cta.tile.bulk_group [%0, {%1, %2, %3}], [%4];" ::"l"(map), "r"(c0),
-               "r"(c1), "r"(c2), "r"(smem_u32(src))
-               : "memory");
-}
-__device__ __forceinline__ void tma_store_commit() { asm volatile("cp.async.bulk.commit_group;" ::: "memory"); }
-__device__ __forceinline__ void tma_store_wait_read() { asm volatile("cp.async.bulk.wait_group.read 0;" ::: "memory"); }
-__device__ __forceinline__ void tma_store_wait_all() { asm volatile("cp.async.bulk.wait_group 0;" ::: "memory"); }
-
-constexpr uint32_t kPeerBitMask = 0xFEFFFFFFu;
-__device__ __forceinline__ uint32_t cluster_ctarank() {
-  uint32_t r;
-  asm volatile("mov.u32 %0, %%cluster_ctarank;" : "=r"(r));
-  return r;
-}
-__device__ __forceinline__ void cluster_sync_all() {
-  asm volatile("barrier.cluster.arrive.release.aligned;" ::: "memory");
-  asm volatile("barrier.cluster.wait.acquire.aligned;" ::: "memory");
-}
-__device__ __forceinline__ void tma_load_2d_2sm(void* dst, const CUtensorMap* map, int c0, int c1, uint64_t* bar) {
-  asm volatile(
-      "cp.async.bulk.tensor.2d.cta_group::2.shared::cluster.global.mbarrier::complete_tx::bytes [%0], [%1, {%2, %3}], [%4];" ::"r"(
-          smem_u32(dst)),
-      "l"(map), "r"(c0), "r"(c1), "r"(smem_u32(bar) & kPeerBitMask)
-      : "memory");
-}
-__device__ __forceinline__ void umma_bf16_2sm(uint32_t tmem_d, uint64_t da, uint64_t db, uint32_t idesc, uint32_t acc) {
-  asm volatile(
-      "{\n\t.reg .pred p;\n\t"
-      "setp.ne.b32 p, %4, 0;\n\t"
-      "tcgen05.mma.cta_group::2.kind::f16 [%0], %1, %2, %3, p;\n\t}" ::"r"(tmem_d),
-      "l"(da), "l"(db), "r"(idesc), "r"(acc)
-      : "memory");
-}
-__device__ __forceinline__ void umma_commit_2sm(uint64_t* bar) {
-  asm volatile("tcgen05.commit.cta_group::2.mbarrier::arrive::one.shared::cluster.multicast::cluster.b64 [%0], %1;" ::"r"(smem_u32(bar)),
-               "h"((uint16_t)3)
-               : "memory");
-}
-__device__ __forceinline__ void mbar_arrive_leader(uint64_t* bar) {
-  asm volatile("mbarrier.arrive.shared::cluster.b64 _, [%0];" ::"r"(smem_u32(bar) & kPeerBitMask) : "memory");
-}
 
 template <int ACT, int BK, int CTAS, bool WRES>
 __global__ void __launch_bounds__(kThreads, 1) gemm_tc_kernel(const __grid_constant__ TcParams p) {
@@ -270,7 +150,7 @@
     }
   } else if (warp == kMmaWarp) {
     if (lane == 0 && leader) {
-      const uint32_t idesc = (1u << 4) | (1u << 7) | (1u << 10) | ((uint32_t)(p.umma_n >> 3) << 17) | ((uint32_t)((BM * CTAS) >> 4) << 24);
+      const uint32_t idesc = umma_idesc_bf16(p.umma_n, BM * CTAS);
       long long it = 0;
       int ti = 0;
       if (WRES && t_first < total_tiles) {
@@ -371,13 +251,7 @@
           if (ACT == ACT_GELU) v[i] = gelu_tanh_fast(v[i]);
         }
         if (p.c_f32 != nullptr || hm_mode) {
-          tma_store_wait_read();
-          __syncwarp();
-#pragma unroll
-          for (int c = 0; c < 8; ++c)
-            *reinterpret_cast<float4*>(stg + lane * 128 + ((c ^ (lane & 7)) << 4)) = make_float4(v[4 * c], v[4 * c + 1], v[4 * c + 2], v[4 * c + 3]);
-          asm volatile("fence.proxy.async.shared::cta;" ::: "memory");
-          __syncwarp();
+          stage_f32_block(stg, lane, v);
           if (lane == 0) {
             if (hm_mode) tma_store_3d(&p.o_hm, oc0, row0, oslab, stg);
             else tma_store_2d(&p.o_f32, oc0, row0, stg);
@@ -385,27 +259,7 @@
           }
         }
         if (p.c_hi != nullptr) {
-          tma_store_wait_read();
-          __syncwarp();
-          uint32_t hi[16], lo[16];
-#pragma unroll
-          for (int i = 0; i < 16; ++i) {
-            __nv_bfloat162 h2, l2;
-            h2.x = __float2bfloat16_rn(v[2 * i]);
-            h2.y = __float2bfloat16_rn(v[2 * i + 1]);
-            l2.x = __float2bfloat16_rn(v[2 * i] - __bfloat162float(h2.x));
-            l2.y = __float2bfloat16_rn(v[2 * i + 1] - __bfloat162float(h2.y));
-            hi[i] = *reinterpret_cast<uint32_t*>(&h2);
-            lo[i] = *reinterpret_cast<uint32_t*>(&l2);
-          }
-#pragma unroll
-          for (int c = 0; c < 4; ++c) {
-            const int off = lane * 64 + ((c ^ ((lane >> 1) & 3)) << 4);
-            *reinterpret_cast<uint4*>(stg + off) = make_uint4(hi[4 * c], hi[4 * c + 1], hi[4 * c + 2], hi[4 * c + 3]);
-            *reinterpret_cast<uint4*>(stg + 2048 + off) = make_uint4(lo[4 * c], lo[4 * c + 1], lo[4 * c + 2], lo[4 * c + 3]);
-          }
-          asm volatile("fence.proxy.async.shared::cta;" ::: "memory");
-          __syncwarp();
+          stage_planes_block(stg, lane, v);
           if (lane == 0) {
             tma_store_2d(&p.o_hi, oc0, row0, stg);
             tma_store_2d(&p.o_lo, oc0, row0, stg + 2048);
@@ -449,6 +303,8 @@
   }
 }
 
+}
+
 typedef CUresult (*EncodeTiledFn)(CUtensorMap*, CUtensorMapDataType, cuuint32_t, void*, const cuuint64_t*, const cuuint64_t*,
                                   const cuuint32_t*, const cuuint32_t*, CUtensorMapInterleave, CUtensorMapSwizzle,
                                   CUtensorMapL2promotion, CUtensorMapFloatOOBfill);
@@ -492,6 +348,11 @@
              CU_TENSOR_MAP_L2_PROMOTION_NONE, CU_TENSOR_MAP_FLOAT_OOB_FILL_NONE) == CUDA_SUCCESS;
 }
 
+int sm_count() {
+  static int sms_c[kMaxDevices] = {0};
+  const int dev = current_device();
+  if (sms_c[dev] == 0 && cudaDeviceGetAttribute(&sms_c[dev], cudaDevAttrMultiProcessorCount, dev) != cudaSuccess) return 148;
+  return sms_c[dev];
 }
 
 bool gemm_tc_available() {
diff --git a/qagnn_b200/csrc/node_mlp.cu b/qagnn_b200/csrc/node_mlp.cu
--- /dev/null
+++ b/qagnn_b200/csrc/node_mlp.cu
@@ -0,0 +1,324 @@
+#include <stdio.h>
+#include <stdlib.h>
+#include <string.h>
+
+#include "tc_sm100.cuh"
+
+namespace qagnn {
+
+namespace {
+
+constexpr int BM = 128, BK = 64, CTAS = 2;
+constexpr int kEpiWarps = 8;
+constexpr int kEpiGroups = kEpiWarps / 4;
+constexpr int kThreads = (kEpiWarps + 2) * 32;
+constexpr int kTmaWarp = kEpiWarps, kMmaWarp = kEpiWarps + 1;
+constexpr int kMaxD = 256;
+constexpr int kMaxKb = (kMaxD + BK - 1) / BK;
+constexpr int kWStages = 3;
+constexpr uint32_t kSlotBytes = 2u * BM * BK * 2;
+constexpr uint32_t kAcc2Col = 256;
+
+struct alignas(64) MlpParams {
+  CUtensorMap a_hi, a_lo, w1_hi, w1_lo, w2_hi, w2_lo;
+  long long M;
+  int D, umma_n, nkb;
+  const float* b1;
+  const float* b2;
+  float* c_f32;
+  __nv_bfloat16 *c_hi, *c_lo;
+  int ldc, ldp;
+};
+
+size_t smem_bytes_for(int D) {
+  const int umma_n = (D + 15) / 16 * 16, nkb = (D + BK - 1) / BK;
+  return (size_t)nkb * kSlotBytes + (size_t)kWStages * 2 * (umma_n / CTAS) * BK * 2 + 1024;
+}
+
+template <int ACT>
+__device__ __forceinline__ void bias_act(float (&v)[32], const float* __restrict__ bias, int c0, int D) {
+  if (c0 + 32 <= D) {
+    const float4* b4 = reinterpret_cast<const float4*>(bias + c0);
+#pragma unroll
+    for (int i = 0; i < 8; ++i) {
+      const float4 b = __ldg(b4 + i);
+      v[4 * i] += b.x; v[4 * i + 1] += b.y; v[4 * i + 2] += b.z; v[4 * i + 3] += b.w;
+    }
+  } else {
+#pragma unroll
+    for (int i = 0; i < 32; ++i) v[i] = c0 + i < D ? v[i] + __ldg(bias + c0 + i) : 0.f;
+  }
+#pragma unroll
+  for (int i = 0; i < 32; ++i) {
+    if (ACT == ACT_RELU) v[i] = fmaxf(v[i], 0.f);
+    if (ACT == ACT_GELU) v[i] = gelu_tanh_fast(v[i]);
+  }
+}
+
+template <int ACT2>
+__global__ void __launch_bounds__(kThreads, 1) node_mlp_tc_kernel(const __grid_constant__ MlpParams p) {
+  extern __shared__ __align__(1024) unsigned char smem[];
+  const int warp = threadIdx.x >> 5, lane = threadIdx.x & 31;
+  const int nkb = p.nkb, D = p.D;
+  const uint32_t plane_bytes = BM * BK * 2;
+  const uint32_t wn = (uint32_t)p.umma_n / CTAS;
+  const uint32_t w_bytes = wn * BK * 2;
+  const uint32_t rank = cluster_ctarank();
+  const bool leader = rank == 0;
+  const unsigned cl_id = blockIdx.x / CTAS, n_cl = gridDim.x / CTAS;
+  unsigned char* region = smem;
+  unsigned char* wring = region + (size_t)nkb * kSlotBytes;
+  unsigned char* ctrl = wring + (size_t)kWStages * 2 * w_bytes;
+  uint64_t* a_full = reinterpret_cast<uint64_t*>(ctrl);
+  uint64_t* a_empty = a_full + kMaxKb;
+  uint64_t* h_full = a_empty + kMaxKb;
+  uint64_t* w_full = h_full + kMaxKb;
+  uint64_t* w_empty = w_full + kWStages;
+  uint64_t* acc1_full = w_empty + kWStages;
+  uint64_t* acc2_full = acc1_full + 1;
+  uint64_t* acc2_empty = acc2_full + 1;
+  uint32_t* tmem_slot = reinterpret_cast<uint32_t*>(acc2_empty + 1);
+
+  const long long total_tiles = (p.M + BM * CTAS - 1) / (BM * CTAS);
+
+  if (threadIdx.x == 0) {
+    for (int kb = 0; kb < kMaxKb; ++kb) {
+      mbar_init(&a_full[kb], 1);
+      mbar_init(&a_empty[kb], 1);
+      mbar_init(&h_full[kb], kEpiWarps * CTAS);
+    }
+    for (int s = 0; s < kWStages; ++s) {
+      mbar_init(&w_full[s], 1);
+      mbar_init(&w_empty[s], 1);
+    }
+    mbar_init(acc1_full, 1);
+    mbar_init(acc2_full, 1);
+    mbar_init(acc2_empty, kEpiWarps * CTAS);
+    asm volatile("fence.mbarrier_init.release.cluster;" ::: "memory");
+  }
+  if (warp == kMmaWarp) {
+    asm volatile("tcgen05.alloc.cta_group::2.sync.aligned.shared::cta.b32 [%0], %1;" ::"r"(smem_u32(tmem_slot)), "r"(512u) : "memory");
+    asm volatile("tcgen05.relinquish_alloc_permit.cta_group::2.sync.aligned;" ::: "memory");
+  }
+  tc_fence_before();
+  __syncthreads();
+  cluster_sync_all();
+  tc_fence_after();
+  const uint32_t tmem_base = *tmem_slot;
+
+  if (warp == kTmaWarp) {
+    if (lane == 0) {
+      long long wit = 0;
+      auto load_w = [&](const CUtensorMap* mh, const CUtensorMap* ml, int kb) {
+        const int s = (int)(wit % kWStages);
+        if (wit >= kWStages) mbar_wait(&w_empty[s], (uint32_t)((wit / kWStages) - 1) & 1u);
+        unsigned char* dst = wring + (size_t)s * 2 * w_bytes;
+        if (leader) mbar_expect_tx(&w_full[s], 2 * 2 * w_bytes);
+        tma_load_2d_2sm(dst, mh, kb * BK, (int)(rank * wn), &w_full[s]);
+        tma_load_2d_2sm(dst + w_bytes, ml, kb * BK, (int)(rank * wn), &w_full[s]);
+        ++wit;
+      };
+      int ti = 0;
+      for (long long tile = cl_id; tile < total_tiles; tile += n_cl, ++ti) {
+        const int m0 = (int)(tile * BM * CTAS + rank * BM);
+        for (int kb = 0; kb < nkb; ++kb) {
+          if (ti > 0) mbar_wait(&a_empty[kb], (uint32_t)(ti - 1) & 1u);
+          unsigned char* dst = region + (size_t)kb * kSlotBytes;
+          if (leader) mbar_expect_tx(&a_full[kb], 2 * kSlotBytes);
+          tma_load_2d_2sm(dst, &p.a_hi, kb * BK, m0, &a_full[kb]);
+          tma_load_2d_2sm(dst + plane_bytes, &p.a_lo, kb * BK, m0, &a_full[kb]);
+          load_w(&p.w1_hi, &p.w1_lo, kb);
+        }
+        for (int kb = 0; kb < nkb; ++kb) load_w(&p.w2_hi, &p.w2_lo, kb);
+      }
+    }
+  } else if (warp == kMmaWarp) {
+    if (lane == 0 && leader) {
+      const uint32_t idesc = umma_idesc_bf16(p.umma_n, BM * CTAS);
+      long long wit = 0;
+      auto mma_kb = [&](uint32_t tmem_d, int kb) {
+        const int s = (int)(wit % kWStages);
+        mbar_wait(&w_full[s], (uint32_t)(wit / kWStages) & 1u);
+        tc_fence_after();
+        const int krem = D - kb * BK;
+        const int nsteps = krem >= BK ? BK / 16 : (krem + 15) / 16;
+        const uint32_t sa = smem_u32(region + (size_t)kb * kSlotBytes);
+        const uint32_t sw = smem_u32(wring + (size_t)s * 2 * w_bytes);
+        for (int k = 0; k < nsteps; ++k) {
+          const uint64_t da_hi = umma_desc<BK>(sa + k * 32), da_lo = umma_desc<BK>(sa + plane_bytes + k * 32);
+          const uint64_t dw_hi = umma_desc<BK>(sw + k * 32), dw_lo = umma_desc<BK>(sw + w_bytes + k * 32);
+          umma_bf16_2sm(tmem_d, da_hi, dw_hi, idesc, (kb | k) != 0);
+          umma_bf16_2sm(tmem_d, da_hi, dw_lo, idesc, 1u);
+          umma_bf16_2sm(tmem_d, da_lo, dw_hi, idesc, 1u);
+        }
+        umma_commit_2sm(&w_empty[s]);
+        ++wit;
+      };
+      int ti = 0;
+      for (long long tile = cl_id; tile < total_tiles; tile += n_cl, ++ti) {
+        const uint32_t par = (uint32_t)ti & 1u;
+        for (int kb = 0; kb < nkb; ++kb) {
+          mbar_wait(&a_full[kb], par);
+          tc_fence_after();
+          mma_kb(tmem_base, kb);
+        }
+        umma_commit_2sm(acc1_full);
+        if (ti > 0) {
+          mbar_wait(acc2_empty, par ^ 1u);
+          tc_fence_after();
+        }
+        for (int kb = 0; kb < nkb; ++kb) {
+          mbar_wait_cluster(&h_full[kb], par);
+          tc_fence_after();
+          mma_kb(tmem_base + kAcc2Col, kb);
+          umma_commit_2sm(&a_empty[kb]);
+        }
+        umma_commit_2sm(acc2_full);
+      }
+    }
+  } else {
+    const int quad = warp & 3, group = warp >> 2;
+    const int r = quad * 32 + lane;
+    const uint32_t tl = (uint32_t)(quad * 32) << 16;
+    int ti = 0;
+    for (long long tile = cl_id; tile < total_tiles; tile += n_cl, ++ti) {
+      const uint32_t par = (uint32_t)ti & 1u;
+      const int row0 = (int)(tile * BM * CTAS + rank * BM) + quad * 32;
+      mbar_wait(acc1_full, par);
+      tc_fence_after();
+      for (int kb = 0; kb < nkb; ++kb) {
+        for (int blk = 2 * kb; blk < 2 * kb + 2; ++blk) {
+          if (blk % kEpiGroups != group || blk * 32 >= D) continue;
+          float v[32];
+          tmem_ld32(tmem_base + tl + (uint32_t)(blk * 32), v);
+          bias_act<ACT_RELU>(v, p.b1, blk * 32, D);
+          uint32_t hi[16], lo[16];
+          split_bf16x32(v, hi, lo);
+          unsigned char* slot = region + (size_t)kb * kSlotBytes + (size_t)r * 128;
+#pragma unroll
+          for (int j = 0; j < 4; ++j) {
+            const int c = (blk & 1) * 4 + j;
+            const int off = (c ^ (r & 7)) << 4;
+            *reinterpret_cast<uint4*>(slot + off) = make_uint4(hi[4 * j], hi[4 * j + 1], hi[4 * j + 2], hi[4 * j + 3]);
+            *reinterpret_cast<uint4*>(slot + plane_bytes + off) = make_uint4(lo[4 * j], lo[4 * j + 1], lo[4 * j + 2], lo[4 * j + 3]);
+          }
+          asm volatile("fence.proxy.async.shared::cta;" ::: "memory");
+        }
+        tc_fence_before();
+        __syncwarp();
+        if (lane == 0) mbar_arrive_leader_release(&h_full[kb]);
+      }
+      mbar_wait(acc2_full, par);
+      tc_fence_after();
+      const long long grow = (long long)row0 + lane;
+      for (int blk = group; blk * 32 < D; blk += kEpiGroups) {
+        const int c0 = blk * 32;
+        float v[32];
+        tmem_ld32(tmem_base + kAcc2Col + tl + (uint32_t)c0, v);
+        bias_act<ACT2>(v, p.b2, c0, D);
+        if (grow < p.M && p.c_f32 != nullptr) {
+          float4* dst = reinterpret_cast<float4*>(p.c_f32 + grow * p.ldc + c0);
+#pragma unroll
+          for (int c = 0; c < 8; ++c)
+            if (c0 + 4 * c < D) dst[c] = make_float4(v[4 * c], v[4 * c + 1], v[4 * c + 2], v[4 * c + 3]);
+        }
+        if (grow < p.M && p.c_hi != nullptr) {
+          uint32_t hi[16], lo[16];
+          split_bf16x32(v, hi, lo);
+          uint4* dh = reinterpret_cast<uint4*>(p.c_hi + grow * p.ldp + c0);
+          uint4* dl = reinterpret_cast<uint4*>(p.c_lo + grow * p.ldp + c0);
+#pragma unroll
+          for (int j = 0; j < 4; ++j)
+            if (c0 + 8 * j < D) {
+              dh[j] = make_uint4(hi[4 * j], hi[4 * j + 1], hi[4 * j + 2], hi[4 * j + 3]);
+              dl[j] = make_uint4(lo[4 * j], lo[4 * j + 1], lo[4 * j + 2], lo[4 * j + 3]);
+            }
+        }
+      }
+      tc_fence_before();
+      __syncwarp();
+      if (lane == 0) mbar_arrive_leader(acc2_empty);
+    }
+  }
+  tc_fence_before();
+  __syncthreads();
+  cluster_sync_all();
+  if (warp == kMmaWarp) {
+    tc_fence_after();
+    asm volatile("tcgen05.dealloc.cta_group::2.sync.aligned.b32 %0, %1;" ::"r"(tmem_base), "r"(512u) : "memory");
+  }
+}
+
+}
+
+bool node_mlp_fused_fits(int D) { return D > 0 && D <= kMaxD && smem_bytes_for(D) <= 227 * 1024; }
+
+int32_t node_mlp_tc(const TcOperand& A, const TcOperand& W1, const float* b1, const TcOperand& W2, const float* b2, long long M,
+                    int D, Act act2, const TcOutput& out, void* hid_hi, void* hid_lo, cudaStream_t st) {
+  if (M <= 0) return QAGNN_OK;
+  if (!gemm_tc_available()) return QAGNN_ERR_UNSUPPORTED;
+  if (!node_mlp_fused_fits(D)) {
+    if (hid_hi == nullptr || hid_lo == nullptr) return QAGNN_ERR_INVALID_ARGUMENT;
+    const TcOperand none{nullptr, nullptr, 0, 0};
+    TcOutput o1{};
+    o1.hi = hid_hi; o1.lo = hid_lo; o1.ldp = D;
+    QAGNN_RETURN_IF(gemm_tc(A, none, W1, b1, M, D, ACT_RELU, o1, st));
+    const TcOperand Hm{hid_hi, hid_lo, D, D};
+    return gemm_tc(Hm, none, W2, b2, M, D, act2, out, st);
+  }
+  if (D % 8 != 0 || A.ld % 8 != 0 || W1.ld % 8 != 0 || W2.ld % 8 != 0) return QAGNN_ERR_UNSUPPORTED;
+  if ((out.f32 && out.ldc % 4 != 0) || (out.hi && out.ldp % 8 != 0) || out.hm_buf != nullptr || out.row_class != nullptr)
+    return QAGNN_ERR_UNSUPPORTED;
+  auto misaligned = [](const void* q) { return ((uintptr_t)q & 15u) != 0; };
+  if (misaligned(out.f32) || misaligned(out.hi) || misaligned(out.lo)) return QAGNN_ERR_UNSUPPORTED;
+  MlpParams p;
+  memset(&p, 0, sizeof(p));
+  p.M = M;
+  p.D = D;
+  p.umma_n = (D + 15) / 16 * 16;
+  p.nkb = (D + BK - 1) / BK;
+  p.b1 = b1;
+  p.b2 = b2;
+  p.c_f32 = out.f32;
+  p.ldc = out.ldc;
+  p.c_hi = (__nv_bfloat16*)out.hi;
+  p.c_lo = (__nv_bfloat16*)out.lo;
+  p.ldp = out.ldp;
+  const int wn = p.umma_n / CTAS;
+  bool ok = make_map(&p.a_hi, A.hi, M, D, A.ld, BM, BK) && make_map(&p.a_lo, A.lo, M, D, A.ld, BM, BK) &&
+            make_map(&p.w1_hi, W1.hi, D, D, W1.ld, wn, BK) && make_map(&p.w1_lo, W1.lo, D, D, W1.ld, wn, BK) &&
+            make_map(&p.w2_hi, W2.hi, D, D, W2.ld, wn, BK) && make_map(&p.w2_lo, W2.lo, D, D, W2.ld, wn, BK);
+  if (!ok) return QAGNN_ERR_CUDA;
+  const size_t smem = smem_bytes_for(D);
+  static bool attr_set[kMaxDevices] = {false};
+  const int dev = current_device();
+  if (!attr_set[dev]) {
+    const int cap = 227 * 1024;
+    QAGNN_CHECK_CUDA(cudaFuncSetAttribute(node_mlp_tc_kernel<ACT_NONE>, cudaFuncAttributeMaxDynamicSharedMemorySize, cap));
+    QAGNN_CHECK_CUDA(cudaFuncSetAttribute(node_mlp_tc_kernel<ACT_RELU>, cudaFuncAttributeMaxDynamicSharedMemorySize, cap));
+    QAGNN_CHECK_CUDA(cudaFuncSetAttribute(node_mlp_tc_kernel<ACT_GELU>, cudaFuncAttributeMaxDynamicSharedMemorySize, cap));
+    attr_set[dev] = true;
+  }
+  const long long tiles = (M + BM * CTAS - 1) / (BM * CTAS);
+  const long long pairs = tiles < sm_count() / CTAS ? tiles : sm_count() / CTAS;
+  cudaLaunchConfig_t cfg;
+  memset(&cfg, 0, sizeof(cfg));
+  cfg.gridDim = dim3((unsigned)(pairs * CTAS));
+  cfg.blockDim = dim3(kThreads);
+  cfg.dynamicSmemBytes = smem;
+  cfg.stream = st;
+  cudaLaunchAttribute lattr[1];
+  lattr[0].id = cudaLaunchAttributeClusterDimension;
+  lattr[0].val.clusterDim.x = CTAS;
+  lattr[0].val.clusterDim.y = 1;
+  lattr[0].val.clusterDim.z = 1;
+  cfg.attrs = lattr;
+  cfg.numAttrs = 1;
+  if (act2 == ACT_NONE) QAGNN_CHECK_CUDA(cudaLaunchKernelEx(&cfg, node_mlp_tc_kernel<ACT_NONE>, p));
+  else if (act2 == ACT_RELU) QAGNN_CHECK_CUDA(cudaLaunchKernelEx(&cfg, node_mlp_tc_kernel<ACT_RELU>, p));
+  else QAGNN_CHECK_CUDA(cudaLaunchKernelEx(&cfg, node_mlp_tc_kernel<ACT_GELU>, p));
+  QAGNN_CHECK_LAUNCH();
+  return QAGNN_OK;
+}
+
+}
diff --git a/qagnn_b200/csrc/tc_sm100.cuh b/qagnn_b200/csrc/tc_sm100.cuh
--- /dev/null
+++ b/qagnn_b200/csrc/tc_sm100.cuh
@@ -0,0 +1,188 @@
+#pragma once
+
+#include <cuda.h>
+#include <cuda_bf16.h>
+
+#include "common.cuh"
+
+namespace qagnn {
+
+__device__ __forceinline__ uint32_t smem_u32(const void* p) { return (uint32_t)__cvta_generic_to_shared(p); }
+
+__device__ __forceinline__ void mbar_init(uint64_t* bar, uint32_t count) {
+  asm volatile("mbarrier.init.shared::cta.b64 [%0], %1;" ::"r"(smem_u32(bar)), "r"(count) : "memory");
+}
+__device__ __forceinline__ void mbar_expect_tx(uint64_t* bar, uint32_t bytes) {
+  asm volatile("mbarrier.arrive.expect_tx.shared::cta.b64 _, [%0], %1;" ::"r"(smem_u32(bar)), "r"(bytes) : "memory");
+}
+__device__ __forceinline__ void mbar_wait(uint64_t* bar, uint32_t parity) {
+  uint32_t done;
+  do {
+    asm volatile(
+        "{\n\t.reg .pred p;\n\t"
+        "mbarrier.try_wait.parity.shared::cta.b64 p, [%1], %2;\n\t"
+        "selp.u32 %0, 1, 0, p;\n\t}"
+        : "=r"(done)
+        : "r"(smem_u32(bar)), "r"(parity)
+        : "memory");
+  } while (!done);
+}
+__device__ __forceinline__ void mbar_wait_cluster(uint64_t* bar, uint32_t parity) {
+  uint32_t done;
+  do {
+    asm volatile(
+        "{\n\t.reg .pred p;\n\t"
+        "mbarrier.try_wait.parity.acquire.cluster.shared::cta.b64 p, [%1], %2;\n\t"
+        "selp.u32 %0, 1, 0, p;\n\t}"
+        : "=r"(done)
+        : "r"(smem_u32(bar)), "r"(parity)
+        : "memory");
+  } while (!done);
+}
+__device__ __forceinline__ void tma_load_2d(void* dst, const CUtensorMap* map, int c0, int c1, uint64_t* bar) {
+  asm volatile(
+      "cp.async.bulk.tensor.2d.shared::cluster.global.tile.mbarrier::complete_tx::bytes [%0], [%1, {%2, %3}], [%4];" ::"r"(
+          smem_u32(dst)),
+      "l"(map), "r"(c0), "r"(c1), "r"(smem_u32(bar))
+      : "memory");
+}
+__device__ __forceinline__ void tc_fence_before() { asm volatile("tcgen05.fence::before_thread_sync;" ::: "memory"); }
+__device__ __forceinline__ void tc_fence_after() { asm volatile("tcgen05.fence::after_thread_sync;" ::: "memory"); }
+
+template <int BK>
+__device__ __forceinline__ uint64_t umma_desc(uint32_t saddr) {
+  const uint32_t lo = ((saddr & 0x3FFFFu) >> 4) | (1u << 16);
+  const uint32_t hi = (uint32_t)(8 * BK * 2 / 16) | (1u << 14) | ((BK == 64 ? 2u : 4u) << 29);
+  return ((uint64_t)hi << 32) | lo;
+}
+__host__ __device__ __forceinline__ uint32_t umma_idesc_bf16(int n, int m) {
+  return (1u << 4) | (1u << 7) | (1u << 10) | ((uint32_t)(n >> 3) << 17) | ((uint32_t)(m >> 4) << 24);
+}
+__device__ __forceinline__ void umma_bf16(uint32_t tmem_d, uint64_t da, uint64_t db, uint32_t idesc, uint32_t acc) {
+  asm volatile(
+      "{\n\t.reg .pred p;\n\t"
+      "setp.ne.b32 p, %4, 0;\n\t"
+      "tcgen05.mma.cta_group::1.kind::f16 [%0], %1, %2, %3, p;\n\t}" ::"r"(tmem_d),
+      "l"(da), "l"(db), "r"(idesc), "r"(acc)
+      : "memory");
+}
+__device__ __forceinline__ void umma_commit(uint64_t* bar) {
+  asm volatile("tcgen05.commit.cta_group::1.mbarrier::arrive::one.shared::cluster.b64 [%0];" ::"r"(smem_u32(bar)) : "memory");
+}
+__device__ __forceinline__ void tmem_ld32(uint32_t taddr, float (&v)[32]) {
+  uint32_t r[32];
+  asm volatile(
+      "tcgen05.ld.sync.aligned.32x32b.x32.b32 "
+      "{%0,%1,%2,%3,%4,%5,%6,%7,%8,%9,%10,%11,%12,%13,%14,%15,%16,%17,%18,%19,%20,%21,%22,%23,%24,%25,%26,%27,%28,%29,%30,%31}, [%32];"
+      : "=r"(r[0]), "=r"(r[1]), "=r"(r[2]), "=r"(r[3]), "=r"(r[4]), "=r"(r[5]), "=r"(r[6]), "=r"(r[7]), "=r"(r[8]),
+        "=r"(r[9]), "=r"(r[10]), "=r"(r[11]), "=r"(r[12]), "=r"(r[13]), "=r"(r[14]), "=r"(r[15]), "=r"(r[16]), "=r"(r[17]),
+        "=r"(r[18]), "=r"(r[19]), "=r"(r[20]), "=r"(r[21]), "=r"(r[22]), "=r"(r[23]), "=r"(r[24]), "=r"(r[25]), "=r"(r[26]),
+        "=r"(r[27]), "=r"(r[28]), "=r"(r[29]), "=r"(r[30]), "=r"(r[31])
+      : "r"(taddr));
+  asm volatile("tcgen05.wait::ld.sync.aligned;" ::: "memory");
+#pragma unroll
+  for (int i = 0; i < 32; ++i) v[i] = __uint_as_float(r[i]);
+}
+
+__device__ __forceinline__ float gelu_tanh_fast(float x) {
+  const float u = 0.7978845608028654f * (x + 0.044715f * x * x * x);
+  const float t = 1.f - __fdividef(2.f, __expf(2.f * u) + 1.f);
+  return 0.5f * x * (1.f + t);
+}
+
+__device__ __forceinline__ void split_bf16x32(const float (&v)[32], uint32_t (&hi)[16], uint32_t (&lo)[16]) {
+#pragma unroll
+  for (int i = 0; i < 16; ++i) {
+    __nv_bfloat162 h2, l2;
+    h2.x = __float2bfloat16_rn(v[2 * i]);
+    h2.y = __float2bfloat16_rn(v[2 * i + 1]);
+    l2.x = __float2bfloat16_rn(v[2 * i] - __bfloat162float(h2.x));
+    l2.y = __float2bfloat16_rn(v[2 * i + 1] - __bfloat162float(h2.y));
+    hi[i] = *reinterpret_cast<uint32_t*>(&h2);
+    lo[i] = *reinterpret_cast<uint32_t*>(&l2);
+  }
+}
+
+constexpr int kStageBytesPerWarp = 4096;
+
+__device__ __forceinline__ void tma_store_2d(const CUtensorMap* map, int c0, int c1, const void* src) {
+  asm volatile("cp.async.bulk.tensor.2d.global.shared::cta.tile.bulk_group [%0, {%1, %2}], [%3];" ::"l"(map), "r"(c0), "r"(c1),
+               "r"(smem_u32(src))
+               : "memory");
+}
+__device__ __forceinline__ void tma_store_3d(const CUtensorMap* map, int c0, int c1, int c2, const void* src) {
+  asm volatile("cp.async.bulk.tensor.3d.global.shared::cta.tile.bulk_group [%0, {%1, %2, %3}], [%4];" ::"l"(map), "r"(c0),
+               "r"(c1), "r"(c2), "r"(smem_u32(src))
+               : "memory");
+}
+__device__ __forceinline__ void tma_store_commit() { asm volatile("cp.async.bulk.commit_group;" ::: "memory"); }
+__device__ __forceinline__ void tma_store_wait_read() { asm volatile("cp.async.bulk.wait_group.read 0;" ::: "memory"); }
+__device__ __forceinline__ void tma_store_wait_all() { asm volatile("cp.async.bulk.wait_group 0;" ::: "memory"); }
+
+__device__ __forceinline__ void stage_f32_block(unsigned char* stg, int lane, const float (&v)[32]) {
+  tma_store_wait_read();
+  __syncwarp();
+#pragma unroll
+  for (int c = 0; c < 8; ++c)
+    *reinterpret_cast<float4*>(stg + lane * 128 + ((c ^ (lane & 7)) << 4)) = make_float4(v[4 * c], v[4 * c + 1], v[4 * c + 2], v[4 * c + 3]);
+  asm volatile("fence.proxy.async.shared::cta;" ::: "memory");
+  __syncwarp();
+}
+__device__ __forceinline__ void stage_planes_block(unsigned char* stg, int lane, const float (&v)[32]) {
+  tma_store_wait_read();
+  __syncwarp();
+  uint32_t hi[16], lo[16];
+  split_bf16x32(v, hi, lo);
+#pragma unroll
+  for (int c = 0; c < 4; ++c) {
+    const int off = lane * 64 + ((c ^ ((lane >> 1) & 3)) << 4);
+    *reinterpret_cast<uint4*>(stg + off) = make_uint4(hi[4 * c], hi[4 * c + 1], hi[4 * c + 2], hi[4 * c + 3]);
+    *reinterpret_cast<uint4*>(stg + 2048 + off) = make_uint4(lo[4 * c], lo[4 * c + 1], lo[4 * c + 2], lo[4 * c + 3]);
+  }
+  asm volatile("fence.proxy.async.shared::cta;" ::: "memory");
+  __syncwarp();
+}
+
+constexpr uint32_t kPeerBitMask = 0xFEFFFFFFu;
+__device__ __forceinline__ uint32_t cluster_ctarank() {
+  uint32_t r;
+  asm volatile("mov.u32 %0, %%cluster_ctarank;" : "=r"(r));
+  return r;
+}
+__device__ __forceinline__ void cluster_sync_all() {
+  asm volatile("barrier.cluster.arrive.release.aligned;" ::: "memory");
+  asm volatile("barrier.cluster.wait.acquire.aligned;" ::: "memory");
+}
+__device__ __forceinline__ void tma_load_2d_2sm(void* dst, const CUtensorMap* map, int c0, int c1, uint64_t* bar) {
+  asm volatile(
+      "cp.async.bulk.tensor.2d.cta_group::2.shared::cluster.global.mbarrier::complete_tx::bytes [%0], [%1, {%2, %3}], [%4];" ::"r"(
+          smem_u32(dst)),
+      "l"(map), "r"(c0), "r"(c1), "r"(smem_u32(bar) & kPeerBitMask)
+      : "memory");
+}
+__device__ __forceinline__ void umma_bf16_2sm(uint32_t tmem_d, uint64_t da, uint64_t db, uint32_t idesc, uint32_t acc) {
+  asm volatile(
+      "{\n\t.reg .pred p;\n\t"
+      "setp.ne.b32 p, %4, 0;\n\t"
+      "tcgen05.mma.cta_group::2.kind::f16 [%0], %1, %2, %3, p;\n\t}" ::"r"(tmem_d),
+      "l"(da), "l"(db), "r"(idesc), "r"(acc)
+      : "memory");
+}
+__device__ __forceinline__ void umma_commit_2sm(uint64_t* bar) {
+  asm volatile("tcgen05.commit.cta_group::2.mbarrier::arrive::one.shared::cluster.multicast::cluster.b64 [%0], %1;" ::"r"(smem_u32(bar)),
+               "h"((uint16_t)3)
+               : "memory");
+}
+__device__ __forceinline__ void mbar_arrive_leader(uint64_t* bar) {
+  asm volatile("mbarrier.arrive.shared::cluster.b64 _, [%0];" ::"r"(smem_u32(bar) & kPeerBitMask) : "memory");
+}
+__device__ __forceinline__ void mbar_arrive_leader_release(uint64_t* bar) {
+  asm volatile("mbarrier.arrive.release.cluster.shared::cluster.b64 _, [%0];" ::"r"(smem_u32(bar) & kPeerBitMask) : "memory");
+}
+
+bool make_map(CUtensorMap* m, const void* base, long long rows, int K, int ld, int box_rows, int BK);
+bool make_out_map(CUtensorMap* m, void* base, int elem_bytes, long long cols, long long rows, long long slabs,
+                  size_t row_stride_bytes, size_t slab_stride_bytes);
+int sm_count();
+
+}
diff --git a/qagnn_b200/ops.py b/qagnn_b200/ops.py
--- a/qagnn_b200/ops.py
+++ b/qagnn_b200/ops.py
@@ -23,3 +23,22 @@
                                      _lib.ptr(out), N, M, N, code, _lib.ptr(ws), nbytes, _lib.stream_ptr(a1.device))
     _lib.check(st, "qagnn_linear_bf16x3")
     return out
+
+
+def node_mlp_bf16x3(a, w1, b1, w2, b2, act="none"):
+    lib = _lib.load()
+    a = _lib.f32c(a, "a")
+    w1, w2 = _lib.f32c(w1, "w1"), _lib.f32c(w2, "w2")
+    b1, b2 = _lib.f32c(b1, "b1"), _lib.f32c(b2, "b2")
+    M, D = a.shape
+    if w1.shape != (D, D) or w2.shape != (D, D) or b1.shape != (D,) or b2.shape != (D,):
+        raise ValueError("w1 / w2 must be [D, D] and b1 / b2 [D] for a of shape [M, D]")
+    out = torch.empty(M, D, dtype=torch.float32, device=a.device)
+    nbytes = lib.qagnn_node_mlp_workspace_bytes(M, D)
+    ws = torch.empty(nbytes, dtype=torch.uint8, device=a.device)
+    code = {"none": 0, "relu": 1, "gelu": 2}[act]
+    with torch.cuda.device(a.device):
+        st = lib.qagnn_node_mlp_bf16x3(_lib.ptr(a), D, _lib.ptr(w1), _lib.ptr(b1), _lib.ptr(w2), _lib.ptr(b2), _lib.ptr(out), D, M,
+                                       D, code, _lib.ptr(ws), nbytes, _lib.stream_ptr(a.device))
+    _lib.check(st, "qagnn_node_mlp_bf16x3")
+    return out
```

Result: slower. 1.012 billion (median of 6 runs) (-3.3%).
